# Gadersd/stable-diffusion-xl-burn

Hardware: AMD Instinct MI355X
Metric: images/sec SDXL-base 1024x1024 30-step CFG7.5 (whole job); UNet step ms p50 (higher is better)
Workload: dtype f16; 1 GPU; SDXL-base 1024x1024, n_steps=30 (31 CFG UNet step pairs), CFG 7.5, batch 1 prompt/GPU + VAE decode to u8 (BASELINE configs[1]); precision=f16, vae_dtype=f32_split, weights=synthetic seeded (random-init SDXL-base architecture), mix_classes=0, parallelism=replica x1, 1 prompt per GPU, weights broadcast once over RCCL, hipgraph=True, split_cfg=False, fused_xattn=True, pipelined_decode=False, prompts_per_call=1, full=False, library=stable-diffusion-xl-burn_amd/lib/libsdxl_mi355.so, debug_set=

## Files before the change

stable-diffusion-xl-burn_amd/csrc/capi_ops.hip:

```cpp
#include "capi_internal.h"
#include <algorithm>
#include <cmath>

using namespace sdxl;

namespace {
__global__ void transpose_pad_kernel(const float* src, int lds_, int rows, int C, void* dst, int dt, int ldd) {
  const size_t i = (size_t)blockIdx.x * blockDim.x + threadIdx.x;
  if (i >= (size_t)rows * C) return;
  const int r = i / C, c = i - (size_t)r * C;
  const float v = src[(size_t)r * lds_ + c];
  if (dt == DT_F16) reinterpret_cast<_Float16*>(dst)[(size_t)c * ldd + r] = (_Float16)v;
  else reinterpret_cast<float*>(dst)[(size_t)c * ldd + r] = v;
}
__global__ void causal_mask_kernel(float* out, int n) {
  const int i = blockIdx.x * blockDim.x + threadIdx.x;
  if (i >= n * n) return;
  const int r = i / n, c = i - r * n;
  out[i] = c > r ? -INFINITY : 0.f;
}

struct Operand { std::string name; std::vector<int> shape; int kind; const float* data = nullptr; float eps = 0.f; int ld = 0; };
using Operands = std::vector<Operand>;
void add_linear(Operands& o, const std::string& n, int K, int N, const float* w, const float* b, int ld = 0) {
// ... 249 lines not shown
  SDXL_REQUIRE(ctx && x && gamma && beta && out, "null argument");
  SDXL_REQUIRE(n_group > 0 && C % n_group == 0, "The number of channels must be divisible by the number of groups");
  SDXL_REQUIRE(C % 8 == 0 && n_group <= 256, "unsupported GroupNorm shape");
  use(ctx);
  hipStream_t s = pick(ctx, stream);
  int cdt, sdt; no_mix(dtype); dtypes(dtype, cdt, sdt); no_split(cdt, "sdxl_group_norm");
  Tmp tmp;
  void* xi = tmp.get((size_t)B * HW * C * dt_size(sdt));
  void* yo = tmp.get((size_t)B * HW * C * dt_size(cdt));
  float* part = (float*)tmp.get(groupnorm_workspace_floats(B, n_group) * sizeof(float));
  launch_nchw_to_nhwc(x, C * HW, xi, sdt, B, C, HW, C, 1.0f, s);
  GroupNormParams p{};
  p.X = xi; p.x_dt = sdt; p.ldx = C; p.Y = yo; p.y_dt = cdt; p.ldy = C; p.gamma = gamma; p.beta = beta; p.partial = part;
  p.B = B; p.HW = HW; p.C = C; p.G = n_group; p.eps = eps; p.silu = silu;
  launch_groupnorm(p, s);
  launch_nhwc_to_nchw(yo, cdt, C, out, B, C, HW, 1.0f, s);
  SDXL_HIP(hipStreamSynchronize(s));
  API_END
}
int sdxl_layer_norm(sdxl_ctx* ctx, void* stream, const float* x, const float* gamma, const float* beta, int rows, int C,
                    float eps, int dtype, float* out) {
  API_BEGIN
  SDXL_REQUIRE(ctx && x && gamma && beta && out, "null argument");
  SDXL_REQUIRE(C % 8 == 0, "unsupported LayerNorm width");
  use(ctx);
  hipStream_t s = pick(ctx, stream);
  int cdt, sdt; no_mix(dtype); dtypes(dtype, cdt, sdt); no_split(cdt, "sdxl_layer_norm");
  Tmp tmp;
  void* xi = tmp.get((size_t)rows * C * dt_size(sdt));
  void* yo = tmp.get((size_t)rows * C * dt_size(cdt));
  launch_copy_rows(x, DT_F32, C, xi, sdt, C, rows, C, s);
  LayerNormParams p{};
  p.X = xi; p.x_dt = sdt; p.ldx = C; p.Y = yo; p.y_dt = cdt; p.ldy = C; p.gamma = gamma; p.beta = beta; p.rows = rows; p.C = C; p.eps = eps;
  launch_layernorm(p, s);
  launch_copy_rows(yo, cdt, C, out, DT_F32, C, rows, C, s);
  SDXL_HIP(hipStreamSynchronize(s));
  API_END
}
int sdxl_conv2d(sdxl_ctx* ctx, void* stream, const float* x, const float* weight, const float* bias, int B, int Cin, int H,
                int W, int Cout, int ksize, int stride, int pad, int upsample, int dtype, float* out) {
  API_BEGIN
  SDXL_REQUIRE(ctx && x && weight && out, "null argument");
  use(ctx);
  hipStream_t s = pick(ctx, stream);
  int cdt, sdt;
  if (dtype == SDXL_DTYPE_F32_SPLIT) { cdt = DT_HL; sdt = DT_HL; }
  else { no_mix(dtype); dtypes(dtype, cdt, sdt); }
  SDXL_REQUIRE(cdt != DT_HL || Cin % 32 == 0, "SDXL_DTYPE_F32_SPLIT convolutions need Cin % 32 == 0");
  const int Hs = upsample ? 2 * H : H, Ws = upsample ? 2 * W : W;
  const int Ho = (Hs + 2 * pad - ksize) / stride + 1, Wo = (Ws + 2 * pad - ksize) / stride + 1;
  Operands ops;
  add_conv(ops, "conv", Cout, Cin, ksize, weight, bias);
  Packed pk(ops, cdt, s);
  const Lin l = pk.wb.conv("conv");
  Tmp tmp;
  void* xi = tmp.get((size_t)B * H * W * Cin * dt_size(sdt));
  float* yo = (float*)tmp.get((size_t)B * Ho * Wo * Cout * sizeof(float));
  Act xa(xi, Cin, sdt);
  if (cdt == DT_HL) {
    float* x32 = (float*)tmp.get((size_t)B * H * W * Cin * sizeof(float));
    float* sc = (float*)tmp.get(hl_scale_floats(B) * sizeof(float));
    launch_nchw_to_nhwc(x, Cin * H * W, x32, DT_F32, B, Cin, H * W, Cin, 1.0f, s);
    launch_f32_to_hl_scaled(x32, Cin, xi, Cin, (size_t)B * H * W, Cin, sc, s, B);
    xa.a_scale = hl_scale_inv(sc, B); xa.a_scale_n = B;
  } else launch_nchw_to_nhwc(x, Cin * H * W, xi, sdt, B, Cin, H * W, Cin, 1.0f, s);
  Exec ex; ex.s = s; ex.cdt = cdt; ex.sdt = sdt;
  give_splitk_ws(ex, tmp, B, Ho * Wo, Cout, s);
  run_conv(ex, l, xa, Cin, ConvGeom{B, H, W, Ho, Wo, ksize, stride, pad, upsample ? 1 : 0}, Act(yo, Cout, DT_F32));
  launch_nhwc_to_nchw(yo, DT_F32, Cout, out, B, Cout, Ho * Wo, 1.0f, s);
  SDXL_HIP(hipStreamSynchronize(s));
  API_END
}
int sdxl_linear(sdxl_ctx* ctx, void* stream, const float* x, const float* weight, const float* bias, int M, int K, int N,
                int geglu, int dtype, float* out) {
  API_BEGIN
  SDXL_REQUIRE(ctx && x && weight && out, "null argument");
  SDXL_REQUIRE(!geglu || (N % 32 == 0), "GEGLU width must be a multiple of 32");
  use(ctx);
  hipStream_t s = pick(ctx, stream);
  int cdt, sdt;
  if (dtype == SDXL_DTYPE_F32_SPLIT) { cdt = DT_HL; sdt = DT_HL; }
  else { no_mix(dtype); dtypes(dtype, cdt, sdt); }
  SDXL_REQUIRE(cdt != DT_HL || K % 32 == 0, "SDXL_DTYPE_F32_SPLIT linear layers need K % 32 == 0");
  Operands ops;
  add_linear(ops, "lin", K, N, weight, bias);
  Packed pk(ops, cdt, s);
  const Lin l = pk.wb.linear("lin", geglu != 0);
  Tmp tmp;
  void* xi = tmp.get((size_t)M * K * dt_size(sdt));
  Act xa(xi, K, sdt);
  if (cdt == DT_HL) {
    float* sc = (float*)tmp.get(hl_scale_floats(1) * sizeof(float));
    launch_f32_to_hl_scaled(x, K, xi, K, (size_t)M, K, sc, s, 1);
    xa.a_scale = hl_scale_inv(sc, 1);
  } else launch_copy_rows(x, DT_F32, K, xi, sdt, K, M, K, s);
  Exec ex; ex.s = s; ex.cdt = cdt; ex.sdt = sdt;
  give_splitk_ws(ex, tmp, 1, M, N, s);
  Epi e; e.act = geglu ? 1 : 0;
  run_linear(ex, l, xa, M, Act(out, geglu ? N / 2 : N, DT_F32), e);
  SDXL_HIP(hipStreamSynchronize(s));
  API_END
}
int sdxl_layer_norm_linear(sdxl_ctx* ctx, void* stream, const float* x, const float* gamma, const float* beta, float eps,
                           const float* weight, const float* bias, int M, int K, int N, int geglu, int dtype, float* out) {
  API_BEGIN
  SDXL_REQUIRE(ctx && x && gamma && beta && weight && out, "null argument");
  SDXL_REQUIRE(!geglu || (N % 32 == 0), "GEGLU width must be a multiple of 32");
// ... 217 lines not shown
```

stable-diffusion-xl-burn_amd/csrc/elementwise.hip:

```cpp
#include "kernels.h"
#include <algorithm>
#include <stdexcept>

namespace sdxl {

typedef _Float16 half_t;
typedef _Float16 half8 __attribute__((ext_vector_type(8)));
typedef float f32x4 __attribute__((ext_vector_type(4)));

__device__ __forceinline__ float ld_f(const void* p, size_t i, int dt) {
  if (dt == DT_HL) { const half_t* b = reinterpret_cast<const half_t*>(p) + ((i >> 4) << 5) + (i & 15); return (float)b[0] + (float)b[16]; }
  return dt == DT_F16 ? (float)reinterpret_cast<const half_t*>(p)[i] : reinterpret_cast<const float*>(p)[i];
}
__device__ __forceinline__ void st_f(void* p, size_t i, int dt, float v) {
  if (dt == DT_HL) {
    half_t* b = reinterpret_cast<half_t*>(p) + ((i >> 4) << 5) + (i & 15);
    const half_t hi = (half_t)v;
    b[0] = hi; b[16] = (half_t)(v - (float)hi);
  } else if (dt == DT_F16) reinterpret_cast<half_t*>(p)[i] = (half_t)v; else reinterpret_cast<float*>(p)[i] = v;
}
__device__ __forceinline__ float silu_f(float x) { return x / (1.0f + expf(-x)); }

template <typename WT>
__global__ __launch_bounds__(256) void gemv_kernel(const GemvParams p, int cols) {
// ... 722 lines not shown
    asm("" : "+v"(w));
    const half_t hi = (half_t)w;
    v = !part ? hi : mode == 0 ? (half_t)((w - (float)hi) * lo_scale) : (half_t)((float)hi / lo_scale);
  }
  dst[i + (size_t)n_offset * 2 * K] = v;
}
void launch_pack_linear_hilo(const float* src, void* dst, int K, int N, int Npad, int geglu, float lo_scale, hipStream_t s, int mode, int n_offset) {
  const size_t total = (size_t)Npad * 2 * K;
  hipLaunchKernelGGL(pack_linear_hilo_kernel, dim3((unsigned)((total + 255) / 256)), dim3(256), 0, s, src, reinterpret_cast<half_t*>(dst), K, N, Npad, geglu, lo_scale, mode, n_offset);
}
__global__ void colsum_packed_kernel(const void* wp, int dt, int Kpad, int nrows, float* cs, const float* kscale, int K, int interleave) {
  const int row = blockIdx.x * 4 + (threadIdx.x >> 6), lane = threadIdx.x & 63;
  if (row >= nrows) return;
  float acc = 0.f;
  if (kscale && interleave) {
    for (int k = lane; k < K; k += 64) acc = fmaf(kscale[k], ld_f(wp, (size_t)row * Kpad + 32 * (k >> 4) + (k & 15), dt), acc);
  } else
  if (kscale) { for (int k = lane; k < K; k += 64) acc = fmaf(kscale[k], ld_f(wp, (size_t)row * Kpad + k, dt), acc); }
  else for (int k = lane; k < Kpad; k += 64) acc += ld_f(wp, (size_t)row * Kpad + k, dt);
#pragma unroll
  for (int o = 32; o > 0; o >>= 1) acc += __shfl_xor(acc, o);
  if (lane == 0) cs[row] = acc;
}
void launch_colsum_packed(const void* wp, int dt, int Kpad, int nrows, float* cs, hipStream_t s, const float* kscale, int K, int interleave) {
  hipLaunchKernelGGL(colsum_packed_kernel, dim3((nrows + 3) / 4), dim3(256), 0, s, wp, dt, Kpad, nrows, cs, kscale, K, interleave);
}
__global__ void beta_dot_kernel(const float* w, const float* beta, const float* bias, float* out, int K, int N) {
  const int n = blockIdx.x * blockDim.x + threadIdx.x;
  if (n >= N) return;
  float acc = bias ? bias[n] : 0.f;
  for (int k = 0; k < K; ++k) acc += beta[k] * w[(size_t)k * N + n];
  out[n] = acc;
}
void launch_beta_dot(const float* w, const float* beta, const float* bias, float* out, int K, int N, hipStream_t s) {
  hipLaunchKernelGGL(beta_dot_kernel, dim3((N + 255) / 256), dim3(256), 0, s, w, beta, bias, out, K, N);
}
__global__ void pack_conv_kernel(const float* src, void* dst, int dt, int Cout, int Cin, int ks, int Kpad, int Npad, float wscale) {
  const size_t i = (size_t)blockIdx.x * blockDim.x + threadIdx.x;
  if (i >= (size_t)Npad * Kpad) return;
  const int n = i / Kpad;
  const int k = i - (size_t)n * Kpad;
  float v = 0.f;
  if (n < Cout && k < ks * ks * Cin) {
    const int tap = k / Cin, c = k - tap * Cin;
    const int ky = tap / ks, kx = tap - ky * ks;
    v = src[(((size_t)n * Cin + c) * ks + ky) * ks + kx] * wscale;
  }
  st_f(dst, i, dt, v);
}
void launch_pack_conv(const float* src, void* dst, int dt, int Cout, int Cin, int ks, int Kpad, int Npad, hipStream_t s, float wscale) {
  const size_t total = (size_t)Npad * Kpad;
  hipLaunchKernelGGL(pack_conv_kernel, dim3((total + 255) / 256), dim3(256), 0, s, src, dst, dt, Cout, Cin, ks, Kpad, Npad, wscale);
}
__global__ void pack_bias_kernel(const float* src, float* dst, int N, int Npad, int geglu, int n_offset) {
  const int i = blockIdx.x * blockDim.x + threadIdx.x;
  if (i >= Npad) return;
  float v = 0.f;
  if (i < N && src) v = src[geglu ? geglu_unpermute(i, N) : i];
  dst[n_offset + i] = v;
}
void launch_pack_bias(const float* src, float* dst, int N, int Npad, int geglu, int n_offset, hipStream_t s) {
  hipLaunchKernelGGL(pack_bias_kernel, dim3((Npad + 255) / 256), dim3(256), 0, s, src, dst, N, Npad, geglu, n_offset);
}

}
```

stable-diffusion-xl-burn_amd/csrc/engine.h:

```cpp
#pragma once
#include "kernels.h"

#include <map>
#include <memory>
#include <stdexcept>
#include <string>
#include <utility>
#include <vector>

namespace sdxl {

struct Error : std::runtime_error {
  explicit Error(const std::string& m) : std::runtime_error(m) {}
};
#define SDXL_HIP(x)                                                                                   \
  do {                                                                                                \
    hipError_t e__ = (x);                                                                             \
    if (e__ != hipSuccess) throw ::sdxl::Error(std::string(#x) + " failed: " + hipGetErrorString(e__)); \
  } while (0)
#define SDXL_REQUIRE(cond, msg)                          \
  do {                                                   \
    if (!(cond)) throw ::sdxl::Error(std::string(msg));  \
  } while (0)

// ... 35 lines not shown
uint64_t fnv1a64(const std::string& s);

struct DeviceArena {
  char* base = nullptr;
  size_t cap = 0, off = 0, peak = 0;
  bool dry = false;
  ~DeviceArena();
  void reserve(size_t bytes);
  void* alloc(size_t bytes);
  size_t mark() const { return off; }
  void reset(size_t m) { off = m; }
};

struct WeightSource {
  virtual ~WeightSource() {}
  virtual void fetch(const ParamSpec& s, size_t index, float* dst_dev, hipStream_t st) = 0;
  virtual bool empty() const { return false; }
};
struct NullSource : WeightSource {
  void fetch(const ParamSpec&, size_t, float*, hipStream_t) override {}
  bool empty() const override { return true; }
};
constexpr float kHiLoScale = 256.0f;
constexpr uint64_t kSeedF16Weights = 1ull << 63;
struct SyntheticSource : WeightSource {
  uint64_t seed;
  explicit SyntheticSource(uint64_t s) : seed(s) {}
  void fetch(const ParamSpec& s, size_t index, float* dst_dev, hipStream_t st) override;
};
struct FlatSource : WeightSource {
  const float* base; std::vector<size_t> offsets;
  FlatSource(const float* b, const std::vector<ParamSpec>& specs);
  void fetch(const ParamSpec& s, size_t index, float* dst_dev, hipStream_t st) override;
};

struct FlatSourceF16 : WeightSource {
  const uint16_t* base; std::vector<size_t> offsets;
  void* stage = nullptr; size_t stage_numel = 0;
  FlatSourceF16(const uint16_t* b, const std::vector<ParamSpec>& specs);
  ~FlatSourceF16() override;
  void fetch(const ParamSpec& s, size_t index, float* dst_dev, hipStream_t st) override;
};

struct Lin {
  const void* w = nullptr; const float* b = nullptr;
  const void* wf = nullptr;
  int N = 0, K = 0, Kpad = 0, Npad = 0, ksize = 1, cin = 0;
  const float* cs = nullptr;
  const float* ln_eps = nullptr;
  int ln_k = 0;
  int k_form = 0;
  int dt = -1;
  const float* acc_scale = nullptr;
};
struct NormW { const float* gamma = nullptr; const float* beta = nullptr; const float* eps = nullptr; int C = 0; };

struct WeightBuilder {
  const std::vector<ParamSpec>& specs;
  std::map<std::string, size_t> index;
  WeightSource& src;
  DeviceArena& arena;
  int dt;
  hipStream_t st;
  float* tmp = nullptr; size_t tmp_numel = 0;
  std::string last_fetched;
  WeightBuilder(const std::vector<ParamSpec>& sp, WeightSource& s, DeviceArena& a, int dtype, hipStream_t stream);
  ~WeightBuilder();
  bool wfrag = true;
  static size_t arena_bound(const std::vector<ParamSpec>& specs, int dt, bool wfrag = true);
  const ParamSpec& spec(const std::string& name, size_t* idx = nullptr) const;
  bool has(const std::string& name) const { return index.count(name) != 0; }
  const float* fetch(const std::string& name);
  Lin linear(const std::string& name, bool geglu = false, int dt_override = -1);
  Lin fused_linear(const std::vector<std::string>& names, int dt_override = -1);
  Lin linear_hilo(const std::string& name, bool geglu, bool dup = false, bool hl_interleave = false);
  float hl_scale(Lin& l, const std::vector<std::string>& weight_names);
  Lin linear_ln(const std::string& name, bool geglu, const std::string& norm, bool xattn_query = false);
  Lin fused_linear_ln(const std::vector<std::string>& names, const std::string& norm);
  Lin fold_ln(const std::vector<std::string>& names, const std::string& norm, bool geglu, int dt_override = -1, bool shadow = false, Lin* plain = nullptr, bool hilo_dup = false,
              bool hl_interleave = false);
  bool all_f16_exact(const std::vector<std::string>& names);
  float* tmp2 = nullptr; size_t tmp2_numel = 0;
  Lin conv(const std::string& name);
  void attach_wfrag(Lin& l, bool fill, bool folded = false);
  NormW norm(const std::string& name);
};

struct Act {
  void* p = nullptr; int ld = 0; int dt = DT_F16;
  const float* gn_part = nullptr; int gn_rt = 0;
  const float* a_scale = nullptr;
  int a_scale_n = 1;
  Act() {}
  Act(void* p_, int ld_, int dt_) : p(p_), ld(ld_), dt(dt_) {}
  Act cols(int c0) const { Act a((char*)p + (size_t)c0 * dt_size(dt), ld, dt); a.a_scale = a_scale; a.a_scale_n = a_scale_n; return a; }
};

struct Profiler {
  enum { IGEMM = 0, ATTENTION = 1, GROUPNORM = 2, LAYERNORM = 3, OTHER = 4, NCLS = 5 };
  struct Rec { hipEvent_t a, b; int cls; double flops; int m, n, k, ks, tag; };
  std::vector<Rec> recs;
  void begin(int cls, double flops, hipStream_t s, int m = 0, int n = 0, int k = 0, int ks = 0, int tag = 0);
  void end(hipStream_t s);
  void collect(float ms[NCLS], int launches[NCLS], double flops[NCLS]);
};

struct WarmSeq {
  struct Item { const void* w; unsigned bytes; bool host; unsigned budget; const void* warm[3]; unsigned warm_bytes[3]; };
  std::vector<Item> seq;
  size_t pos = 0;
  bool recording = false, ready = false;
  void finish();
};
struct Exec {
  Profiler* prof = nullptr;
  hipStream_t s = nullptr;
  bool dry = false;
  int cdt = DT_F16;
  int sdt = DT_F16;
  DeviceArena* act = nullptr;
  float* gn_partial = nullptr;
  float* splitk_ws = nullptr; size_t splitk_ws_bytes = 0; unsigned* splitk_cnt = nullptr;
  const float* ebias = nullptr;
  int b0 = 0;
  hipEvent_t fork_ev = nullptr;
  int fork_after = 0, launches = 0;
  WarmSeq* warm = nullptr;
  float* attn_xws = nullptr; unsigned* attn_xcnt = nullptr;
  int demote = 0;
  Act alloc(size_t rows, int C, int dt) {
    return Act(act->alloc(rows * (size_t)C * dt_size(dt)), C, dt);
  }
};

enum MixClass {
  MIX_ATTN_F16 = 1,
// ... 285 lines not shown
```

stable-diffusion-xl-burn_amd/csrc/igemm_common.h:

```cpp
#pragma once
#include "kernels.h"
#include <stdexcept>
#include <type_traits>

namespace sdxl {

typedef _Float16 half_t;
typedef _Float16 half8 __attribute__((ext_vector_type(8)));
typedef _Float16 half4 __attribute__((ext_vector_type(4)));
typedef float f32x4 __attribute__((ext_vector_type(4)));
typedef float f32x16 __attribute__((ext_vector_type(16)));

typedef const __attribute__((address_space(1))) void* gptr_t;
typedef float f32x8 __attribute__((ext_vector_type(8)));
__device__ __forceinline__ f32x8 uniform_load8(const float* ptr) {
  const unsigned long long a = (unsigned long long)(uintptr_t)ptr;
  const unsigned long long u = ((unsigned long long)__builtin_amdgcn_readfirstlane((unsigned)(a >> 32)) << 32) | (unsigned)__builtin_amdgcn_readfirstlane((unsigned)a);
  return *(const __attribute__((address_space(4))) f32x8*)(uintptr_t)u;
}
__device__ __forceinline__ f32x4 col_vec4(const float* arr, bool present, int nbu, int fh, const void* zeros) {
  const f32x8 c = uniform_load8(present ? arr + nbu : reinterpret_cast<const float*>(zeros));
  return fh ? f32x4{c[4], c[5], c[6], c[7]} : f32x4{c[0], c[1], c[2], c[3]};
}
typedef __attribute__((address_space(3))) void* lptr_t;
// ... 67 lines not shown
  static constexpr int TPR = NT / BM;
  static constexpr bool OK = NT % BM == 0 && (TPR == 2 || TPR == 4);
  static constexpr int NC = OK ? 4 / TPR : 1, PERC = 6;
  ln_f32x2 v[NC][PERC];
  int row, sub;
  bool live;
  __device__ __forceinline__ void load(const IgemmParams& p, int m0, int tid) {
    row = tid / TPR; sub = tid - row * TPR;
    const int m = m0 + row;
    live = p.ln_stat != nullptr && p.ln_slots <= 24;
    const ln_f32x2* st = reinterpret_cast<const ln_f32x2*>(p.ln_stat) + (m < p.M ? m : 0);
    const size_t M = (size_t)p.M;
#pragma unroll
    for (int c = 0; c < NC; ++c)
#pragma unroll
      for (int q = 0; q < PERC; ++q) {
        const int k = sub + c * TPR + 4 * q;
        v[c][q] = (live && k < p.ln_slots) ? st[(size_t)k * M] : ln_f32x2{0.f, 0.f};
      }
  }
  __device__ __forceinline__ static float combine(const float (&P)[NC]) {
    if constexpr (TPR == 4) { const float t = P[0] + __shfl_xor(P[0], 1); return t + __shfl_xor(t, 2); }
    else { const float u = P[0] + __shfl_xor(P[0], 1), w = P[1] + __shfl_xor(P[1], 1); return u + w; }
  }
  __device__ __forceinline__ void finish(const IgemmParams& p, int m0, float* coef) {
    if (!live) return;
    float P[NC];
#pragma unroll
    for (int c = 0; c < NC; ++c) {
      P[c] = 0.f;
#pragma unroll
      for (int q = 0; q < PERC; ++q) if (sub + c * TPR + 4 * q < p.ln_slots) P[c] += v[c][q][0];
    }
    const float mu = combine(P) / (float)p.ln_slots;
    float Q[NC], D[NC];
#pragma unroll
    for (int c = 0; c < NC; ++c) {
      Q[c] = 0.f; D[c] = 0.f;
#pragma unroll
      for (int q = 0; q < PERC; ++q)
        if (sub + c * TPR + 4 * q < p.ln_slots) { const float d = v[c][q][0] - mu; Q[c] += v[c][q][1]; D[c] = fmaf(d, d, D[c]); }
    }
    const float s2 = combine(Q), sd = combine(D);
    const float var = (s2 + 64.f * sd) * p.ln_invc;
    const float a = 1.0f / sqrtf(var + (p.ln_eps_ptr ? *p.ln_eps_ptr : p.ln_eps));
    if (sub == 0) {
      const bool ok = m0 + row < p.M;
      coef[row * 2] = ok ? a : 1.f;
      coef[row * 2 + 1] = ok ? -a * mu : 0.f;
    }
  }
};

template <int TM, int TN>
__device__ __forceinline__ void igemm_epilogue(const IgemmParams& p, const f32x16 (&acc)[TM][TN], int mw, int nw, int fr, int fh,
                                               const float (&lnA)[TM], const float (&lnC)[TM]) {
  const bool geglu = p.act == 1;
  const int nlim = geglu ? (p.N >> 1) : p.N;
#pragma unroll
  for (int i = 0; i < TM; ++i) {
    const int m = mw + i * 32 + fr;
    if (m >= p.M) continue;
    const int bidx = m / p.rpb;
    const int key = m - bidx * p.rpb;
    const float lna = lnA[i], lnc = lnC[i];
#pragma unroll
    for (int j = 0; j < TN; ++j) {
      const int nt = nw + j * 32;
#pragma unroll
      for (int q = 0; q < 4; ++q) {
        if (geglu && q >= 2) continue;
        const int nb = nt + 8 * q + 4 * fh;
        if (nb >= p.N) continue;
        float v[4];
#pragma unroll
        for (int r = 0; r < 4; ++r) v[r] = acc[i][j][q * 4 + r];
        if (p.ln_stat) {
          const f32x4 cz = *reinterpret_cast<const f32x4*>(p.ln_cs + nb);
#pragma unroll
          for (int r = 0; r < 4; ++r) v[r] = lna * v[r] + lnc * cz[r];
        }
        if (p.bias) {
          const f32x4 bz = *reinterpret_cast<const f32x4*>(p.bias + nb);
#pragma unroll
          for (int r = 0; r < 4; ++r) v[r] += bz[r];
        }
        if (p.ebias) {
          const f32x4 ez = *reinterpret_cast<const f32x4*>(p.ebias + (size_t)bidx * p.ebias_ld + nb);
#pragma unroll
          for (int r = 0; r < 4; ++r) v[r] += ez[r];
        }
        int nout = nb;
        if (geglu) {
          f32x4 gz = {0.f, 0.f, 0.f, 0.f};
          if (p.bias) gz = *reinterpret_cast<const f32x4*>(p.bias + nb + 16);
          f32x4 gc = {0.f, 0.f, 0.f, 0.f};
          if (p.ln_stat) gc = *reinterpret_cast<const f32x4*>(p.ln_cs + nb + 16);
#pragma unroll
          for (int r = 0; r < 4; ++r) v[r] *= gelu_erf2(lna * acc[i][j][(q + 2) * 4 + r] + lnc * gc[r] + gz[r]);
          nout = (nt >> 1) + 8 * q + 4 * fh;
        }
        if (geglu || nb < p.n_split) {
          const bool vec = nout + 3 < nlim && (nout & 3) == 0;
          if (p.R) {
            if (vec && p.r_dt == DT_F16 && (p.ldr & 3) == 0) {
              const half4 rr = *reinterpret_cast<const half4*>(reinterpret_cast<const half_t*>(p.R) + (size_t)m * p.ldr + nout);
// ... 11 lines not shown
                                           : reinterpret_cast<const float*>(p.R)[(size_t)m * p.ldr + nout + r];
            }
          }
          if (vec && p.c_dt == DT_F16 && (p.ldc & 3) == 0) {
            half4 h; h[0] = (half_t)v[0]; h[1] = (half_t)v[1]; h[2] = (half_t)v[2]; h[3] = (half_t)v[3];
            *reinterpret_cast<half4*>(reinterpret_cast<half_t*>(p.C) + (size_t)m * p.ldc + nout) = h;
          } else if (vec && p.c_dt == DT_F32 && (p.ldc & 3) == 0) {
            f32x4 o = {v[0], v[1], v[2], v[3]};
            *reinterpret_cast<f32x4*>(reinterpret_cast<float*>(p.C) + (size_t)m * p.ldc + nout) = o;
          } else {
#pragma unroll
            for (int r = 0; r < 4; ++r)
              if (nout + r < nlim) {
                if (p.c_dt == DT_F16) reinterpret_cast<half_t*>(p.C)[(size_t)m * p.ldc + nout + r] = (half_t)v[r];
                else reinterpret_cast<float*>(p.C)[(size_t)m * p.ldc + nout + r] = v[r];
              }
          }
        } else {
#pragma unroll
          for (int r = 0; r < 4; ++r)
            if (nb + r < p.N) {
              const size_t o = ((size_t)bidx * p.ct_rows + (nb + r - p.n_split)) * p.ct_ld + key;
              if (p.c_dt == DT_F16) reinterpret_cast<half_t*>(p.Ct)[o] = (half_t)v[r];
              else reinterpret_cast<float*>(p.Ct)[o] = v[r];
            }
        }
      }
    }
  }
}

__host__ __device__ constexpr int pipe_lds_total(int ring, int extra) { return ring + extra + 2048 <= 163840 ? ring + extra + 2048 : ring + extra; }

typedef int warm_i32x4 __attribute__((ext_vector_type(4)));
template <int NT>
__device__ __forceinline__ void igemm_warm_body(const void* base, unsigned bytes, int wi, int nw) {
  const char* b = reinterpret_cast<const char*>(base);
  constexpr unsigned span = NT * 16, step = span * 8;
  warm_i32x4 acc = {0, 0, 0, 0};
  for (size_t off = (size_t)wi * step; off < bytes; off += (size_t)nw * step) {
    warm_i32x4 v[8];
#pragma unroll
    for (int u = 0; u < 8; ++u) {
      const size_t o = off + (size_t)u * span + (size_t)threadIdx.x * 16;
      v[u] = o + 16 <= bytes ? *reinterpret_cast<const warm_i32x4*>(b + o) : warm_i32x4{0, 0, 0, 0};
    }
#pragma unroll
    for (int u = 0; u < 8; ++u) acc ^= v[u];
  }
  asm volatile("" ::"v"(acc));
}

struct GnCtx { char* scratch; int wave, wm, wn, m0, n0; };
template <int TM, int TN, bool GEGLU>
__device__ __forceinline__ void igemm_epilogue_staged_impl(const IgemmParams& p, const f32x16 (&acc)[TM][TN], int mw, int nw,
                                                           int lane, char* lds, bool transposed, const float (&lnA)[TM],
                                                           const float (&lnC)[TM], const void* zeros, const GnCtx* gc = nullptr) {
  constexpr int WM = TM * 32, WN = TN * 32;
  constexpr int ROWS = WM;
  constexpr int COLS = GEGLU ? WN / 2 : WN;
  constexpr int SWN = (COLS % 32) == 0 ? 7 : 0;
  constexpr int SWT = (WM % 32) == 0 ? 7 : 0;
  const int fr = lane & 31, fh = lane >> 5;
  const f32x4* zv = reinterpret_cast<const f32x4*>(zeros);
  constexpr int NQ = GEGLU ? 2 : 4;
  if (!transposed) {
    constexpr int RB = COLS * 4;
    int bidx[TM];
#pragma unroll
    for (int i = 0; i < TM; ++i) { const int m = mw + i * 32 + fr; bidx[i] = (p.ebias && m < p.M) ? m / p.rpb : 0; }
#pragma unroll
    for (int j = 0; j < TN; ++j) {
      const int nt = nw + j * 32;
      f32x4 bz[NQ], cz[NQ], gz[NQ], gc[NQ], ez[TM][NQ];
#pragma unroll
      for (int q = 0; q < NQ; ++q) {
        const int nb = nt + 8 * q + 4 * fh;
        const bool ok = nb < p.N;
        bz[q] = *((p.bias && ok) ? reinterpret_cast<const f32x4*>(p.bias + nb) : zv);
        cz[q] = *((p.ln_stat && ok) ? reinterpret_cast<const f32x4*>(p.ln_cs + nb) : zv);
        if constexpr (GEGLU) {
          gz[q] = *((p.bias && ok) ? reinterpret_cast<const f32x4*>(p.bias + nb + 16) : zv);
          gc[q] = *((p.ln_stat && ok) ? reinterpret_cast<const f32x4*>(p.ln_cs + nb + 16) : zv);
        }
#pragma unroll
        for (int i = 0; i < TM; ++i)
          ez[i][q] = *((p.ebias && ok) ? reinterpret_cast<const f32x4*>(p.ebias + (size_t)bidx[i] * p.ebias_ld + nb) : zv);
      }
#pragma unroll
      for (int i = 0; i < TM; ++i) {
        const int row = i * 32 + fr;
        const float lna = lnA[i], lnc = lnC[i];
#pragma unroll
        for (int q = 0; q < NQ; ++q) {
          f32x4 v;
#pragma unroll
          for (int r = 0; r < 4; ++r) v[r] = acc[i][j][q * 4 + r];
          v = lna * v + lnc * cz[q] + bz[q] + ez[i][q];
          int col = j * 32 + 8 * q + 4 * fh;
          if constexpr (GEGLU) {
#pragma unroll
            for (int r = 0; r < 4; ++r) v[r] *= gelu_erf2(lna * acc[i][j][(q + 2) * 4 + r] + lnc * gc[q][r] + gz[q][r]);
            col = j * 16 + 8 * q + 4 * fh;
          }
          *reinterpret_cast<f32x4*>(lds + row * RB + ((((col >> 2) ^ (row & SWN))) << 4)) = v;
        }
      }
    }
  } else {
    constexpr int RB = WM * 4;
// ... 65 lines not shown
    for (int it = 0; it < NIT; ++it) {
      const int idx = it * 64 + lane;
      const int row = idx / LPR, piece = idx - row * LPR;
      const int n0 = nwo + piece * 8;
      const int m = mw + row;
      const half_t* rp = reinterpret_cast<const half_t*>(p.R) + (size_t)m * p.ldr + n0;
      rfast[it] = p.R && p.r_dt == DT_F16 && idx < ITEMS && m < p.M && n0 + 8 <= nlim && (reinterpret_cast<uintptr_t>(rp) & 15) == 0;
      rpre[it] = *(rfast[it] ? reinterpret_cast<const half8*>(rp) : reinterpret_cast<const half8*>(zeros));
    }
#pragma unroll
    for (int it = 0; it < NIT; ++it) {
      const int idx = it * 64 + lane;
      const int row = idx / LPR, piece = idx - row * LPR;
      if (ITEMS % 64 != 0 && idx >= ITEMS) continue;
      const int n0 = nwo + piece * 8;
      const int m = mw + row;
      const f32x4 a = *reinterpret_cast<const f32x4*>(lds + row * RB + (((2 * piece) ^ (row & SWN)) << 4));
      const f32x4 b = *reinterpret_cast<const f32x4*>(lds + row * RB + (((2 * piece + 1) ^ (row & SWN)) << 4));
      const bool valid = m < p.M && n0 < nlim;
      float rr[8] = {0.f, 0.f, 0.f, 0.f, 0.f, 0.f, 0.f, 0.f};
      if (valid) {
      float v[8] = {a[0], a[1], a[2], a[3], b[0], b[1], b[2], b[3]};
      const bool full = n0 + 8 <= nlim;
      if (rfast[it]) {
#pragma unroll
        for (int e = 0; e < 8; ++e) v[e] += (float)rpre[it][e];
      } else if (p.R) {
        if (p.r_dt == DT_F16) {
          const half_t* rp = reinterpret_cast<const half_t*>(p.R) + (size_t)m * p.ldr + n0;
          if (full && (reinterpret_cast<uintptr_t>(rp) & 15) == 0) {
            const half8 rr = *reinterpret_cast<const half8*>(rp);
#pragma unroll
            for (int e = 0; e < 8; ++e) v[e] += (float)rr[e];
          } else {
#pragma unroll
            for (int e = 0; e < 8; ++e) if (n0 + e < nlim) v[e] += (float)rp[e];
          }
        } else {
          const float* rp = reinterpret_cast<const float*>(p.R) + (size_t)m * p.ldr + n0;
          if (full && (reinterpret_cast<uintptr_t>(rp) & 15) == 0) {
            const f32x4 r0 = *reinterpret_cast<const f32x4*>(rp), r1 = *reinterpret_cast<const f32x4*>(rp + 4);
#pragma unroll
            for (int e = 0; e < 4; ++e) { v[e] += r0[e]; v[4 + e] += r1[e]; }
          } else {
#pragma unroll
            for (int e = 0; e < 8; ++e) if (n0 + e < nlim) v[e] += rp[e];
          }
        }
      }
      if (p.stat_out || gnp) {
#pragma unroll
        for (int e = 0; e < 8; ++e) rr[e] = p.c_dt == DT_F16 ? (float)(half_t)v[e] : v[e];
      }
      if (p.c_dt == DT_F16) {
        half_t* cp = reinterpret_cast<half_t*>(p.C) + (size_t)m * p.ldc + n0;
        if (full && (reinterpret_cast<uintptr_t>(cp) & 15) == 0) {
          half8 h;
#pragma unroll
          for (int e = 0; e < 8; ++e) h[e] = (half_t)v[e];
          *reinterpret_cast<half8*>(cp) = h;
        } else {
#pragma unroll
          for (int e = 0; e < 8; ++e) if (n0 + e < nlim) cp[e] = (half_t)v[e];
        }
      } else if (p.c_dt == DT_HL) {
        if (full) store_hl8(reinterpret_cast<float*>(p.C) + (size_t)m * p.ldc, n0, v);
      } else {
        float* cp = reinterpret_cast<float*>(p.C) + (size_t)m * p.ldc + n0;
        if (full && (reinterpret_cast<uintptr_t>(cp) & 15) == 0) {
          *reinterpret_cast<f32x4*>(cp) = f32x4{v[0], v[1], v[2], v[3]};
          *reinterpret_cast<f32x4*>(cp + 4) = f32x4{v[4], v[5], v[6], v[7]};
        } else {
#pragma unroll
          for (int e = 0; e < 8; ++e) if (n0 + e < nlim) cp[e] = v[e];
        }
      }
      }
      if constexpr (GNP) {
        if (gnp) {
          if (it == 0) {
#pragma unroll
            for (int e = 0; e < 8; ++e) gpiv[e] = __shfl(rr[e], lane & 7);
          }
#pragma unroll
          for (int e = 0; e < 8; ++e) { const float d = rr[e] - gpiv[e]; gs1[e] += d; gs2[e] = fmaf(d, d, gs2[e]); }
        }
      }
      if constexpr (COLS % 64 == 0) {
        if (p.stat_out) {
          const float piv = __shfl(rr[0], lane & ~7);
          float s1 = 0.f, s2 = 0.f;
#pragma unroll
          for (int e = 0; e < 8; ++e) { const float d = rr[e] - piv; s1 += d; s2 = fmaf(d, d, s2); }
          st_piv[it] = piv; st_s1[it] = s1; st_s2[it] = s2;
          st_ok[it] = (piece & 7) == 0 && valid;
          st_off[it] = ((size_t)(n0 >> 6) * p.M + m) * 2;
        }
      }
    }
    if constexpr (COLS % 64 == 0) {
      if (p.stat_out) {
#pragma unroll
        for (int o = 1; o < 8; o <<= 1) {
#pragma unroll
          for (int it = 0; it < NIT; ++it) { st_s1[it] += __shfl_xor(st_s1[it], o); st_s2[it] += __shfl_xor(st_s2[it], o); }
        }
#pragma unroll
        for (int it = 0; it < NIT; ++it)
          if (st_ok[it]) {
            float* dst = p.stat_out + st_off[it];
            dst[0] = st_piv[it] + st_s1[it] * (1.0f / 64.0f);
            dst[1] = fmaxf(st_s2[it] - st_s1[it] * st_s1[it] * (1.0f / 64.0f), 0.f);
          }
      }
    }
    if constexpr (GNP) {
      if (gnp) {
#pragma unroll
        for (int e = 0; e < 8; ++e) {
#pragma unroll
          for (int o = 8; o < 64; o <<= 1) { gs1[e] += __shfl_xor(gs1[e], o); gs2[e] += __shfl_xor(gs2[e], o); }
// ... 225 lines not shown
          dst[1] = fmaxf(s2 - s1 * s1 * (1.0f / 64.0f), 0.f);
        }
      }
    }
  }
}

template <int TM, int TN>
__device__ __forceinline__ void igemm_epilogue_swapped(const IgemmParams& p, const f32x16 (&acc)[TM][TN], int mw, int nw, int lane,
                                                       const float* coef, const void* zeros) {
  (void)zeros;
  const int fr = lane & 31, fh = lane >> 5;
  const int b = mw / p.rpb;
  const int key_w = mw - b * p.rpb;
#pragma unroll
  for (int j = 0; j < TN; ++j) {
    const int n = nw + j * 32 + fr;
    const float bias = p.bias ? p.bias[n] : 0.f;
    const float cs = p.ln_stat ? p.ln_cs[n] : 0.f;
    half_t* crow = reinterpret_cast<half_t*>(p.Ct) + ((size_t)b * p.ct_rows + (n - p.n_split)) * p.ct_ld + key_w;
#pragma unroll
    for (int i = 0; i < TM; ++i) {
      f32x4 v[4];
#pragma unroll
      for (int g = 0; g < 4; ++g) {
        f32x4 a4 = {1.f, 1.f, 1.f, 1.f}, c4 = {0.f, 0.f, 0.f, 0.f};
        if (coef && p.ln_stat) {
          const f32x4 c01 = *reinterpret_cast<const f32x4*>(coef + (i * 32 + 8 * g + 4 * fh) * 2);
          const f32x4 c23 = *reinterpret_cast<const f32x4*>(coef + (i * 32 + 8 * g + 4 * fh) * 2 + 4);
          a4 = f32x4{c01[0], c01[2], c23[0], c23[2]};
          c4 = f32x4{c01[1], c01[3], c23[1], c23[3]};
        }
#pragma unroll
        for (int r = 0; r < 4; ++r) v[g][r] = __builtin_fmaf(a4[r], acc[i][j][4 * g + r], __builtin_fmaf(c4[r], cs, bias));
      }
#pragma unroll
      for (int t = 0; t < 2; ++t) {
        float w[8];
#pragma unroll
        for (int r = 0; r < 4; ++r) {
          const auto sw = __builtin_amdgcn_permlane32_swap(__float_as_uint(v[2 * t][r]), __float_as_uint(v[2 * t + 1][r]), false, false);
          w[r] = __uint_as_float(sw[0]);
          w[4 + r] = __uint_as_float(sw[1]);
        }
        half8 h;
#pragma unroll
        for (int e = 0; e < 8; ++e) h[e] = (half_t)w[e];
        if (n < p.N) *reinterpret_cast<half8*>(crow + i * 32 + 16 * t + 8 * fh) = h;
      }
    }
  }
}

template <int TM, int TN>
__device__ __forceinline__ void igemm_epilogue_staged(const IgemmParams& p, const f32x16 (&acc)[TM][TN], int mw, int nw,
                                                      int lane, char* lds, const float (&lnA)[TM], const float (&lnC)[TM],
                                                      const void* zeros, const GnCtx* gc = nullptr) {
  constexpr int WN = TN * 32;
  if (p.act == 1) { igemm_epilogue_staged_impl<TM, TN, true>(p, acc, mw, nw, lane, lds, false, lnA, lnC, zeros); return; }
  const bool all_normal = nw + WN <= p.n_split || p.n_split >= p.N;
  const bool all_transposed = nw >= p.n_split;
  if (all_normal) igemm_epilogue_staged_impl<TM, TN, false>(p, acc, mw, nw, lane, lds, false, lnA, lnC, zeros, gc);
  else if (all_transposed) igemm_epilogue_staged_impl<TM, TN, false>(p, acc, mw, nw, lane, lds, true, lnA, lnC, zeros);
  else igemm_epilogue<TM, TN>(p, acc, mw, nw, lane & 31, lane >> 5, lnA, lnC);
}

template <int N, typename F> __device__ __forceinline__ void static_for(F&& f) {
  if constexpr (N > 0) {
    static_for<N - 1>(f);
    f(std::integral_constant<int, N - 1>{});
  }
}
template <int OFF, typename F = half8> __device__ __forceinline__ F lds_read128(unsigned addr) {
  F v;
  asm volatile("ds_read_b128 %0, %1 offset:%2" : "=v"(v) : "v"(addr), "n"(OFF));
  return v;
}
template <typename T> struct PipeElem;
template <> struct PipeElem<half_t> {
  typedef half8 frag;
  static __device__ __forceinline__ f32x16 mma(const half8& w, const half8& a, const f32x16& c) {
    return __builtin_amdgcn_mfma_f32_32x32x16_f16(w, a, c, 0, 0, 0);
  }
};
template <> struct PipeElem<float> {
  typedef f32x4 frag;
  static __device__ __forceinline__ f32x16 mma(const f32x4& w, const f32x4& a, f32x16 c) {
    c = __builtin_amdgcn_mfma_f32_32x32x2f32(w[0], a[0], c, 0, 0, 0);
    c = __builtin_amdgcn_mfma_f32_32x32x2f32(w[1], a[1], c, 0, 0, 0);
    c = __builtin_amdgcn_mfma_f32_32x32x2f32(w[2], a[2], c, 0, 0, 0);
    c = __builtin_amdgcn_mfma_f32_32x32x2f32(w[3], a[3], c, 0, 0, 0);
    return c;
  }
};
template <> struct PipeElem<hl16_t> { typedef half8 frag; };
template <int N> __device__ __forceinline__ void wait_lgkmcnt() {
  asm volatile("s_waitcnt lgkmcnt(%0)" ::"n"(N) : "memory");
  __builtin_amdgcn_sched_barrier(0);
}

__device__ __forceinline__ void xattn_load_frags(const IgemmParams& p, int mw, int nw, int lane, half8 (&kf)[3][4], half8 (&vf)[2][6]) {
  const int mclamp = mw < p.M ? mw : p.M - 1;
  const int b = __builtin_amdgcn_readfirstlane(mclamp / p.rpb);
  const int head = (nw < p.N ? nw : 0) >> 6;
  const half8* fx = reinterpret_cast<const half8*>(p.xa_k) + ((size_t)b * (p.N >> 6) + head) * (24 * 64) + lane;
#pragma unroll
  for (int t = 0; t < 3; ++t)
#pragma unroll
    for (int s4 = 0; s4 < 4; ++s4) kf[t][s4] = fx[(t * 4 + s4) * 64];
#pragma unroll
  for (int dt = 0; dt < 2; ++dt)
// ... 237 lines not shown
```

stable-diffusion-xl-burn_amd/csrc/igemm_glds.hip:

```cpp
#include "igemm_common.h"
#include <atomic>

namespace sdxl {

template <int BM, int BN, int NS, int MINB = 2>
__global__ __launch_bounds__(256, MINB) void igemm_glds_kernel(const IgemmParams p, const void* zeros) {
  kernarg_prefetch<(int)sizeof(IgemmParams) + 8>();
  constexpr int WM = BM / 2, WN = BN / 2;
  constexpr int TM = WM / 32, TN = WN / 32;
  constexpr int AJ = BM / 32, BJ = BN / 32;
  constexpr int PER = AJ + BJ;
  constexpr int KT = 64;
  constexpr int STAGE = (BM + BN) * 128;
  extern __shared__ __attribute__((aligned(16))) char smem[];

  const int tid = threadIdx.x, lane = tid & 63;
  const int wave = __builtin_amdgcn_readfirstlane(tid >> 6);
  const int wm = wave >> 1, wn = wave & 1;

  const int tilesN = (p.N + BN - 1) / BN;
  const int nwg = gridDim.x;
  int bid = blockIdx.x;
  {
    const int q = nwg >> 3, r = nwg & 7, xcd = bid & 7, idx = bid >> 3;
// ... 67 lines not shown
  f32x16 acc[TM][TN];
#pragma unroll
  for (int i = 0; i < TM; ++i)
#pragma unroll
    for (int j = 0; j < TN; ++j)
#pragma unroll
      for (int r = 0; r < 16; ++r) acc[i][j][r] = 0.f;

  const int nk = p.Kpad / KT;
  const int fr = lane & 31, fh = lane >> 5;
#pragma unroll
  for (int s = 0; s < NS - 1; ++s)
    if (s < nk) stage(s);
  float lnA[TM], lnC[TM];
  ln_prologue<TM>(p, m0 + wm * WM, fr, lnA, lnC);
  int cur = 0;
  int nxt = NS - 1;
  for (int kt = 0; kt < nk; ++kt) {
    if (kt + NS - 2 < nk) wait_vmcnt<PER * (NS - 2)>(); else wait_vmcnt<0>();
    asm volatile("" ::: "memory");
    __builtin_amdgcn_s_barrier();
    asm volatile("" ::: "memory");
    if (kt + NS - 1 < nk) stage(nxt);
    const char* a = smem + cur * STAGE;
    const char* b = a + BM * 128;
#pragma unroll
    for (int kk = 0; kk < 4; ++kk) {
      const int ch = kk * 2 + fh;
      half8 fa[TM], fb[TN];
#pragma unroll
      for (int i = 0; i < TM; ++i) {
        const int row = wm * WM + i * 32 + fr;
        fa[i] = *reinterpret_cast<const half8*>(a + row * 128 + ((ch ^ ((row >> 1) & 7)) << 4));
      }
#pragma unroll
      for (int j = 0; j < TN; ++j) {
        const int row = wn * WN + j * 32 + fr;
        fb[j] = *reinterpret_cast<const half8*>(b + row * 128 + ((ch ^ ((row >> 1) & 7)) << 4));
      }
#pragma unroll
      for (int i = 0; i < TM; ++i)
#pragma unroll
        for (int j = 0; j < TN; ++j)
          acc[i][j] = __builtin_amdgcn_mfma_f32_32x32x16_f16(fb[j], fa[i], acc[i][j], 0, 0, 0);
    }
    nxt = cur;
    cur = cur + 1 == NS ? 0 : cur + 1;
  }

  __syncthreads();
  igemm_epilogue_staged<TM, TN>(p, acc, m0 + wm * WM, n0 + wn * WN, lane, smem + wave * (WM * WN * 4), lnA, lnC, zeros);
}

template <int BM, int BN, int NS, int WGM = 4, int NW = 8, typename T = half_t, bool XA = false, bool S2 = false, bool TSW = false, bool XH = false>
__global__ __launch_bounds__(64 * NW) void igemm_pipe_kernel(const IgemmParams p, const void* zeros) {
  kernarg_prefetch<(int)sizeof(IgemmParams) + 8>();
  typedef typename PipeElem<T>::frag frag_t;
  constexpr int CE = 16 / (int)sizeof(T);
  constexpr int WGN = NW / WGM;
  constexpr int WM = BM / WGM, WN = BN / WGN;
  constexpr int TM = WM / 32, TN = WN / 32;
  constexpr int NF = TM + TN;
  constexpr int BPC = BN / 8;
  constexpr int AJ = BM / (8 * NW), BJ = (BPC + NW - 1) / NW;
  constexpr int REM = BPC % NW;
  constexpr int PER = AJ + BJ;
  static_assert(BM % (8 * NW) == 0 && WM % 32 == 0 && WN % 32 == 0 && BN % 8 == 0, "bad tile");
  constexpr int KT = 8 * CE;
  constexpr int STAGE = (BM + BN) * 128;
  constexpr bool LIN = XA;
  static_assert(NS >= 3, "counted-wait pipeline needs a ring of at least 3 slots");
  static_assert(BM * 128 + (TN - 1) * 4096 < 65536, "fragment offsets must fit the ds_read immediate");
  extern __shared__ __attribute__((aligned(16))) char smem[];
  const unsigned lds0 = (unsigned)(uintptr_t)(lptr_t)smem;

  const int tid = threadIdx.x, lane = tid & 63;
  const int wave = __builtin_amdgcn_readfirstlane(tid >> 6);
  const int wm = wave / WGN, wn = wave % WGN;
  const bool lastb = REM == 0 || wave < REM;

  const int tilesN = (p.N + BN - 1) / BN;
  const int tilesM = (p.M + BM - 1) / BM;
  const int nwg = gridDim.x;
  int bid = blockIdx.x;
  {
    const int q = nwg >> 3, r = nwg & 7, xcd = bid & 7, idx = bid >> 3;
    bid = (xcd < r ? xcd * (q + 1) : r * (q + 1) + (xcd - r) * q) + idx;
  }
  const int SK = p.splitk > 1 ? p.splitk : 1;
  const int slice = SK > 1 ? bid % SK : 0;
  if (SK > 1) bid /= SK;
  const int tile_id = bid;
  int tm, tn;
  if ((size_t)p.N * p.K > (size_t)p.M * p.Cin) { tn = bid / tilesM; tm = bid - tn * tilesM; }
  else { tm = bid / tilesN; tn = bid - tm * tilesN; }
  const int m0 = tm * BM, n0 = tn * BN;
  bool tsw_swapped = false;
  if constexpr (TSW) {
    const int ok = n0 >= p.n_split && n0 + BN <= p.N && p.c_dt == DT_F16 && p.act == 0 && !p.epi_staged && (p.rpb % BM) == 0 && m0 + BM <= p.M &&
                   (p.ct_ld & 7) == 0 && (reinterpret_cast<uintptr_t>(p.Ct) & 15) == 0 && (!p.ln_stat || p.ln_slots <= 24);
    tsw_swapped = __builtin_amdgcn_readfirstlane(ok) != 0;
  }
  auto wait_tiles = [&](auto KK) {
    constexpr int k = decltype(KK)::value;
    if constexpr (REM == 0) wait_vmcnt<PER * k>();
    else { if (lastb) wait_vmcnt<PER * k>(); else wait_vmcnt<(PER - 1) * k>(); }
  };

  const int lrow = lane >> 3, slot = lane & 7;
  const T* wptr[BJ];
#pragma unroll
  for (int j = 0; j < BJ; ++j) {
    const int row = (j * NW + wave) * 8 + lrow;
    wptr[j] = reinterpret_cast<const T*>(p.W) + (size_t)(n0 + row) * p.Kpad + (slot ^ ((row >> 1) & 7)) * CE;
  }
  const int nk_all = p.Kpad / KT;
  const int kbeg = SK > 1 ? (int)((long)slice * nk_all / SK) : 0;
  const int nk = SK > 1 ? (int)((long)(slice + 1) * nk_all / SK) - kbeg : nk_all;
  if (kbeg > 0) {
#pragma unroll
    for (int j = 0; j < BJ; ++j) wptr[j] += kbeg * KT;
  }
  constexpr bool B0_EARLY = !LIN;
  if constexpr (B0_EARLY) {
    if (nk > 0) {
      char* lb0 = smem + BM * 128 + wave * 1024;
      static_for<BJ>([&](auto J) {
        constexpr int j = decltype(J)::value;
        if (j < BJ - 1 || lastb) {
          __builtin_amdgcn_global_load_lds((gptr_t)wptr[j], (lptr_t)(lb0 + j * (NW * 1024)), 16, 0, 0);
          wptr[j] += KT;
        }
      });
      __builtin_amdgcn_sched_barrier(0);
    }
  }
  const int HWo = p.Hout * p.Wout;
  const int Hup = p.Hin << p.up, Wup = p.Win << p.up;
  const bool lin_rows = p.ksize == 1 && p.stride == 1 && p.up == 0 && p.pad == 0;
  const bool pow2 = (HWo & (HWo - 1)) == 0 && (p.Wout & (p.Wout - 1)) == 0;
  const int sh_hw = __builtin_ctz((unsigned)HWo | 0x40000000u), sh_w = __builtin_ctz((unsigned)p.Wout | 0x40000000u);
  int rb[AJ], ry[AJ], rx[AJ], rsw[AJ];
#pragma unroll
  for (int j = 0; j < AJ; ++j) {
    const int row = (j * NW + wave) * 8 + lrow;
    const int m = m0 + row;
    rsw[j] = (slot ^ ((row >> 1) & 7)) * CE;
    rb[j] = m < p.M ? m : -1; ry[j] = 0; rx[j] = 0;
    if (!lin_rows) {
      if (m < p.M) {
        int b, rem, oy;
        if (pow2) { b = m >> sh_hw; rem = m & (HWo - 1); oy = rem >> sh_w; }
        else { b = m / HWo; rem = m - b * HWo; oy = rem / p.Wout; }
        rb[j] = b; ry[j] = oy * p.stride - p.pad; rx[j] = (rem - oy * p.Wout) * p.stride - p.pad;
      } else { rb[j] = -1; ry[j] = -(1 << 28); rx[j] = 0; }
    }
  }
  const T* Ag = reinterpret_cast<const T*>(p.A);
  const T* aptr[AJ];
  int aadv[AJ];
  int s_c0 = 0, s_dy = 0, s_dx = 0;
  if (kbeg > 0) {
    const int e0 = kbeg * KT, tap = e0 / p.Cin;
    s_c0 = e0 - tap * p.Cin; s_dy = tap / p.ksize; s_dx = tap - s_dy * p.ksize;
  }
  auto retap = [&]() {
    if (lin_rows) {
#pragma unroll
      for (int j = 0; j < AJ; ++j) {
        const bool ok = rb[j] >= 0 && s_dy == 0;
        aptr[j] = ok ? Ag + (size_t)rb[j] * p.lda + rsw[j] + s_c0 : reinterpret_cast<const T*>(zeros);
        aadv[j] = ok ? KT : 0;
      }
      return;
    }
#pragma unroll
    for (int j = 0; j < AJ; ++j) {
      const int iy = ry[j] + s_dy, ix = rx[j] + s_dx;
      const bool ok = (unsigned)iy < (unsigned)Hup && (unsigned)ix < (unsigned)Wup;
      const size_t off = (((size_t)(rb[j] < 0 ? 0 : rb[j]) * p.Hin + ((ok ? iy : 0) >> p.up)) * p.Win + ((ok ? ix : 0) >> p.up)) * p.lda + rsw[j] + s_c0;
      aptr[j] = ok ? Ag + off : reinterpret_cast<const T*>(zeros);
      aadv[j] = ok ? KT : 0;
    }
  };
  retap();
  unsigned long long abase = 0, wbase = 0;
  unsigned aoff[AJ], woff[BJ];
  if constexpr (LIN) {
    abase = (unsigned long long)(uintptr_t)(Ag + (size_t)m0 * p.lda + (size_t)kbeg * KT);
    wbase = (unsigned long long)(uintptr_t)(reinterpret_cast<const T*>(p.W) + (size_t)n0 * p.Kpad + (size_t)kbeg * KT);
    abase = ((unsigned long long)__builtin_amdgcn_readfirstlane((unsigned)(abase >> 32)) << 32) | (unsigned)__builtin_amdgcn_readfirstlane((unsigned)abase);
    wbase = ((unsigned long long)__builtin_amdgcn_readfirstlane((unsigned)(wbase >> 32)) << 32) | (unsigned)__builtin_amdgcn_readfirstlane((unsigned)wbase);
#pragma unroll
    for (int j = 0; j < AJ; ++j) {
      int row = (j * NW + wave) * 8 + lrow;
      const int sw = (slot ^ ((row >> 1) & 7)) * 16;
      if (m0 + row >= p.M) row = p.M - 1 - m0;
      aoff[j] = (unsigned)row * (unsigned)(p.lda * (int)sizeof(T)) + sw;
    }
#pragma unroll
    for (int j = 0; j < BJ; ++j) {
      const int row = (j * NW + wave) * 8 + lrow;
      woff[j] = (unsigned)row * (unsigned)(p.Kpad * (int)sizeof(T)) + (slot ^ ((row >> 1) & 7)) * 16;
    }
  }
  auto issue = [&](int buf, auto PH) {
    constexpr int ph = decltype(PH)::value;
// ... 241 lines not shown
  if constexpr (HL) {
    wait_lgkmcnt<0>();
    if (hl_wexact) kloop(std::true_type{}); else kloop(std::false_type{});
  } else if constexpr (TSW) {
    wait_lgkmcnt<0>();
    if (tsw_swapped) kloop(std::true_type{}); else kloop(std::false_type{});
  } else kloop(std::false_type{});
  __builtin_amdgcn_s_barrier();
  asm volatile("" ::: "memory");
  if constexpr (BN == 128) {
    if (SK > 1) {
      constexpr int NV = TM * TN * 4;
      f32x4* slab = reinterpret_cast<f32x4*>(p.splitk_ws) + ((size_t)tile_id * SK + slice) * (size_t)(NW * NV * 64);
      static_for<TM * TN>([&](auto X) {
        constexpr int x = decltype(X)::value, i = x / TN, j = x % TN;
#pragma unroll
        for (int q = 0; q < 4; ++q) {
          const f32x4 v = f32x4{acc[i][j][4 * q], acc[i][j][4 * q + 1], acc[i][j][4 * q + 2], acc[i][j][4 * q + 3]};
          f32x4* dst = slab + (size_t)((wave * NV + x * 4 + q) * 64 + lane);
          if (p.splitk_wt) asm volatile("global_store_dwordx4 %0, %1, off sc0 sc1\n\ts_nop 1" ::"v"(dst), "v"(v) : "memory");
          else *dst = v;
        }
      });
      asm volatile("s_waitcnt vmcnt(0)" ::: "memory");
      __syncthreads();
      volatile int* flag = reinterpret_cast<volatile int*>(smem + NS * STAGE - 16);
      if (tid == 0) {
        if (!p.splitk_wt) __builtin_amdgcn_fence(__ATOMIC_RELEASE, "agent");
        asm volatile("s_waitcnt vmcnt(0)" ::: "memory");
        const unsigned t = __hip_atomic_fetch_add(p.splitk_cnt + tile_id, 1u, __ATOMIC_RELAXED, __HIP_MEMORY_SCOPE_AGENT);
        const int last = t == (unsigned)(SK - 1);
        if (last) {
          __hip_atomic_store(p.splitk_cnt + tile_id, 0u, __ATOMIC_RELAXED, __HIP_MEMORY_SCOPE_AGENT);
          __builtin_amdgcn_fence(__ATOMIC_ACQUIRE, "agent");
        }
        *flag = last;
      }
      __syncthreads();
      if (!*flag) return;
      const f32x4* s0 = reinterpret_cast<const f32x4*>(p.splitk_ws) + (size_t)tile_id * SK * (size_t)(NW * NV * 64);
      static_for<TM * TN>([&](auto X) {
        constexpr int x = decltype(X)::value, i = x / TN, j = x % TN;
#pragma unroll
        for (int q = 0; q < 4; ++q) {
          f32x4 sum = s0[(size_t)((wave * NV + x * 4 + q) * 64 + lane)];
          for (int sl = 1; sl < SK; ++sl) sum += s0[(size_t)sl * (NW * NV * 64) + (size_t)((wave * NV + x * 4 + q) * 64 + lane)];
#pragma unroll
          for (int r = 0; r < 4; ++r) acc[i][j][4 * q + r] = sum[r];
        }
      });
      __syncthreads();
    }
  }
  if constexpr (XA) {
    static_assert(TN == 2 && sizeof(T) == 2, "fused cross-attention: wave tile = one 64-wide head, f16");
    static_assert(NW * WM * WN * 4 <= NS * STAGE, "staging regions must fit the dead ring");
    if constexpr (XH) {
      static_assert(!XH || (XA && TM == 1), "split-precision fused cross-attention: XA kernels with one-MFMA-row wave tiles");
      xattn_inplace_hl<TM>(p, acc, m0 + wm * WM, n0 + wn * WN, lane, lnA, lnC, zeros);
    } else {
    if constexpr (!XA_EARLY) xattn_load_frags(p, m0 + wm * WM, n0 + wn * WN, lane, xkf, xvf);
    xattn_inplace<TM>(p, acc, m0 + wm * WM, n0 + wn * WN, lane, lnA, lnC, zeros, xkf, xvf);
    }
    IgemmParams pe = p;
    pe.bias = nullptr; pe.ln_stat = nullptr;
    if (!p.epi_staged && igemm_rows_ok<TM, TN, false>(pe, n0 + wn * WN))
      igemm_epilogue_rows<TM, TN, false>(pe, acc, m0 + wm * WM, n0 + wn * WN, lane, lnA, lnC, zeros);
    else
      igemm_epilogue_staged<TM, TN>(pe, acc, m0 + wm * WM, n0 + wn * WN, lane, smem + wave * (WM * WN * 4), lnA, lnC, zeros);
    return;
  }
  if constexpr (TSW) {
    if (tsw_swapped) {
      igemm_epilogue_swapped<TM, TN>(p, acc, m0 + wm * WM, n0 + wn * WN, lane, ln_coop ? ln_coef + (wm * WM) * 2 : nullptr, zeros);
      return;
    }
  }
  if (!p.epi_staged && p.act != 1 && igemm_rows_ok<TM, TN, false>(p, n0 + wn * WN)) {
    igemm_epilogue_rows<TM, TN, false>(p, acc, m0 + wm * WM, n0 + wn * WN, lane, lnA, lnC, zeros);
    return;
  }
  constexpr bool FITS = NW * WM * WN * 4 <= NS * STAGE;
  if (FITS || p.act == 1) {
    const int region = p.act == 1 ? WM * (WN / 2) * 4 : WM * WN * 4;
    if constexpr (BM == 256 && BN == 128 && NW == 8 && WGM == 4 && (sizeof(T) == 2 || HL)) {
      static_assert(NW * WM * WN * 4 + 4096 <= NS * STAGE, "GroupNorm-statistics scratch must fit behind the staging regions");
      const GnCtx gc{smem + NW * WM * WN * 4, wave, wm, wn, m0, n0};
      igemm_epilogue_staged<TM, TN>(p, acc, m0 + wm * WM, n0 + wn * WN, lane, smem + wave * region, lnA, lnC, zeros, &gc);
    } else
    igemm_epilogue_staged<TM, TN>(p, acc, m0 + wm * WM, n0 + wn * WN, lane, smem + wave * region, lnA, lnC, zeros);
  } else {
    igemm_epilogue<TM, TN>(p, acc, m0 + wm * WM, n0 + wn * WN, fr, fh, lnA, lnC);
  }
}

#ifdef SDXL_MEASURE
__device__ unsigned* g_wide_tl = nullptr;
void igemm_set_wide_timeline(void* buf) {
  unsigned* b = reinterpret_cast<unsigned*>(buf);
  if (hipMemcpyToSymbol(HIP_SYMBOL(g_wide_tl), &b, sizeof(b)) != hipSuccess) throw std::runtime_error("igemm: cannot set the wide-kernel timeline buffer");
}
#define WIDE_STAMP(i) do { wtl[i] = (unsigned)__builtin_amdgcn_s_memtime(); } while (0)
#else
#define WIDE_STAMP(i) do { } while (0)
#endif
template <int NS, bool DB = false>
// ... 177 lines not shown
  }
  WIDE_STAMP(3);
  __builtin_amdgcn_s_barrier();
  asm volatile("" ::: "memory");
  WIDE_STAMP(4);
  if (p.act == 1) {
    char* region = smem + wave * (32 * (WN / 2) * 4);
    {
      const float la1[1] = {lnA[0]}, lc1[1] = {lnC[0]};
      igemm_epilogue_staged_impl<1, TN, true>(p, acc0, m0 + wm * WM, n0 + wn * WN, lane, region, false, la1, lc1, zeros);
    }
    WIDE_STAMP(5);
    {
      const float la1[1] = {lnA[1]}, lc1[1] = {lnC[1]};
      igemm_epilogue_staged_impl<1, TN, true>(p, acc1, m0 + wm * WM + 32, n0 + wn * WN, lane, region, false, la1, lc1, zeros);
    }
  }
#ifdef SDXL_MEASURE
  WIDE_STAMP(6);
  asm volatile("s_waitcnt vmcnt(0)" ::: "memory");
  WIDE_STAMP(7);
  wtl[9] = (unsigned)__builtin_amdgcn_s_memrealtime();
  if (g_wide_tl && lane == 0) {
#pragma unroll
    for (int i = 0; i < 10; ++i) g_wide_tl[((size_t)blockIdx.x * 8 + wave) * 16 + i] = wtl[i];
  }
#endif
}

static const void* g_zero_pages[kMaxDevices] = {};
static int current_device() {
  int d = 0;
  if (hipGetDevice(&d) != hipSuccess || d < 0 || d >= kMaxDevices) throw std::runtime_error("igemm: no current HIP device");
  return d;
}
const void* igemm_zero_page() { return g_zero_pages[current_device()]; }
int igemm_current_device() { return current_device(); }
void igemm_glds_init() {
  const int d = current_device();
  if (g_zero_pages[d]) return;
  void* z = nullptr;
  if (hipMalloc(&z, 4096) != hipSuccess || hipMemset(z, 0, 4096) != hipSuccess)
    throw std::runtime_error("igemm: cannot allocate the zero page");
  g_zero_pages[d] = z;
}

template <int BM, int BN, int NS, int MINB = 2>
static void launch_glds(const IgemmParams& p, const IgemmChoice& c, hipStream_t s) {
  const int dev = current_device();
  set_max_dynamic_lds<&igemm_glds_kernel<BM, BN, NS, MINB>>(c.lds, dev);
  hipLaunchKernelGGL((igemm_glds_kernel<BM, BN, NS, MINB>), dim3(c.grid), dim3(c.block), c.lds, s, p, g_zero_pages[dev]);
}

template <int BM, int BN, int NS, int WGM = 4, int NW = 8, typename T = half_t, bool XA = false, bool S2 = false, bool TSW = false, bool XH = false>
static void launch_pipe(const IgemmParams& p, const IgemmChoice& c, hipStream_t s) {
  if (c.lds != pipe_lds_total(NS * (BM + BN) * 128, 0) || c.block != 64 * NW) throw std::logic_error("igemm: choice and kernel disagree on the LDS layout");
  const int dev = current_device();
  set_max_dynamic_lds<&igemm_pipe_kernel<BM, BN, NS, WGM, NW, T, XA, S2, TSW, XH>>(c.lds, dev);
  if (c.splitk > 1 && (size_t)c.grid * BM * BN * 4 > p.splitk_ws_bytes) throw std::runtime_error("igemm: split-K workspace too small");
  hipLaunchKernelGGL((igemm_pipe_kernel<BM, BN, NS, WGM, NW, T, XA, S2, TSW, XH>), dim3(c.grid), dim3(c.block), c.lds, s, p, g_zero_pages[dev]);
}

static void launch_wide(const IgemmParams& p, const IgemmChoice& c, hipStream_t s) {
  const int dev = current_device();
#ifdef SDXL_MEASURE
  if (c.db) {
    set_max_dynamic_lds<&igemm_wide_kernel<3, true>>(c.lds, dev);
    hipLaunchKernelGGL((igemm_wide_kernel<3, true>), dim3(c.grid), dim3(c.block), c.lds, s, p, g_zero_pages[dev]);
    return;
  }
#endif
  set_max_dynamic_lds<&igemm_wide_kernel<3, false>>(c.lds, dev);
  hipLaunchKernelGGL((igemm_wide_kernel<3, false>), dim3(c.grid), dim3(c.block), c.lds, s, p, g_zero_pages[dev]);
}

__global__ void xattn_pack_kernel(const half_t* K, const half_t* Vt, half8* out, int B, int C, int nctx, int vt_ld) {
  const size_t i = (size_t)blockIdx.x * blockDim.x + threadIdx.x;
  const int H = C >> 6;
  if (i >= (size_t)B * H * 24 * 64) return;
  const int lane = (int)(i & 63), f = (int)((i >> 6) % 24);
  const int bh = (int)(i / (24 * 64)), b = bh / H, h = bh - b * H;
  const int fr = lane & 31, fh = lane >> 5;
  half8 v;
#pragma unroll
  for (int e = 0; e < 8; ++e) {
    const int sub = 8 * (e >> 2) + 4 * fh + (e & 3);
    half_t x = (half_t)0.f;
    if (f < 12) {
      const int key = 32 * (f >> 2) + fr, d = 16 * (f & 3) + sub;
      if (key < nctx) x = K[((size_t)b * nctx + key) * C + h * 64 + d];
    } else {
      const int g = f - 12, d = 32 * (g / 6) + fr, key = 16 * (g % 6) + sub;
      if (key < nctx) x = Vt[((size_t)b * C + h * 64 + d) * vt_ld + key];
    }
    v[e] = x;
  }
  out[i] = v;
}
size_t xattn_pack_bytes(int B, int C) { return (size_t)B * (C / 64) * 24 * 64 * 16; }
void launch_xattn_pack(const void* K, const void* Vt, void* out, int B, int C, int nctx, int vt_ld, hipStream_t s) {
  const size_t n = (size_t)B * (C / 64) * 24 * 64;
  hipLaunchKernelGGL(xattn_pack_kernel, dim3((unsigned)((n + 255) / 256)), dim3(256), 0, s, reinterpret_cast<const half_t*>(K),
                     reinterpret_cast<const half_t*>(Vt), reinterpret_cast<half8*>(out), B, C, nctx, vt_ld);
}

void launch_igemm_dma(const IgemmParams& p, const IgemmChoice& c, hipStream_t s) {
#define PIPE(BM, BN, NS, WGM, NW, T, DT, XA, S2, TSW, XH)                                                                                 \
  if (c.family == IG_PIPE && c.bm == BM && c.bn == BN && c.ns == NS && c.wgm == WGM && c.nw == NW && c.elem == DT && c.xa == XA && c.s2 == S2 && c.tsw == TSW && c.xh == XH) \
    return launch_pipe<BM, BN, NS, WGM, NW, T, XA, S2, TSW, XH>(p, c, s)
  PIPE(96, 128, 3, 3, 6, half_t, DT_F16, true, false, false, true);
  PIPE(128, 128, 4, 4, 8, half_t, DT_F16, true, false, false, true);
  PIPE(256, 128, 3, 4, 8, half_t, DT_F16, true, false, false, false);
  PIPE(128, 128, 4, 4, 8, half_t, DT_F16, true, false, false, false);
  PIPE(128, 128, 5, 4, 8, half_t, DT_F16, true, false, false, false);
  PIPE(96, 128, 3, 3, 6, half_t, DT_F16, true, false, false, false);
  PIPE(256, 128, 3, 4, 8, half_t, DT_F16, false, false, false, false);
  if (c.family == IG_GLDS && c.bm == 128 && c.bn == 128 && c.ns == 2) return launch_glds<128, 128, 2>(p, c, s);
  if (c.family == IG_GLDS && c.bm == 64 && c.bn == 128 && c.ns == 2) return launch_glds<64, 128, 2>(p, c, s);
  PIPE(256, 128, 3, 4, 8, half_t, DT_F16, false, false, true, false);
  PIPE(128, 128, 4, 4, 8, half_t, DT_F16, false, false, false, false);
  PIPE(256, 160, 3, 8, 8, half_t, DT_F16, false, false, false, false);
  PIPE(128, 128, 5, 4, 8, half_t, DT_F16, false, false, false, false);
  PIPE(96, 128, 5, 3, 6, half_t, DT_F16, false, false, false, false);
  PIPE(96, 128, 4, 3, 6, half_t, DT_F16, false, false, false, false);
  PIPE(96, 128, 5, 3, 6, half_t, DT_F16, false, true, false, false);
  PIPE(128, 160, 3, 4, 4, half_t, DT_F16, false, false, false, false);
  if (c.family == IG_WIDE && c.bm == 256 && c.bn == 320 && c.ns == 3) return launch_wide(p, c, s);
  PIPE(256, 128, 3, 4, 8, float, DT_F32, false, false, false, false);
  PIPE(128, 128, 4, 4, 8, float, DT_F32, false, false, false, false);
  PIPE(96, 128, 5, 3, 6, hl16_t, DT_HL, false, false, false, false);
  PIPE(256, 128, 3, 4, 8, hl16_t, DT_HL, false, false, false, false);
  PIPE(128, 160, 3, 4, 4, hl16_t, DT_HL, false, false, false, false);
  PIPE(128, 128, 4, 4, 8, hl16_t, DT_HL, false, false, false, false);
#undef PIPE
  throw std::logic_error("igemm: the selection chose a direct-to-LDS kernel that is not instantiated");
}

}
```

stable-diffusion-xl-burn_amd/csrc/kernels.h:

```cpp
#pragma once
#include <hip/hip_runtime.h>
#include <stdint.h>
#include <stdexcept>

namespace sdxl {

enum DType : int { DT_F32 = 0, DT_F16 = 1, DT_HL = 2 };

static inline size_t dt_size(int dt) { return dt == DT_F16 ? 2 : 4; }

struct IgemmParams {
  const void* A;
  const void* W;
  const void* Wf;
  int a_dt;
  int B, Hin, Win, Cin, lda;
  int Hout, Wout;
  int ksize, stride, pad, up;
  int M, N, K, Kpad;
  const float* bias;
  const float* ebias;
  int ebias_ld;
  int rpb;
  int act;
  const void* R; int ldr; int r_dt;
  void* C; int ldc; int c_dt;
  int n_split;
  void* Ct; int ct_rows; int ct_ld;
  const float* ln_stat; int ln_slots; const float* ln_cs; float ln_invc; float ln_eps;
  const float* ln_eps_ptr;
  float* stat_out; int stat_slots;
  float* splitk_ws; size_t splitk_ws_bytes; unsigned* splitk_cnt; int splitk;
  const void* xa_k; int xa_nctx; float xa_scale;
  const void* xa_k_lo;
  float* gn_part;
  const float* acc_scale;
  const float* a_scale;
  int a_scale_rpb;
  int hl_wexact_ok;
  int xa_vec64;
  const void* warm[3]; unsigned warm_bytes[3];
  int splitk_wt;
  int wreg_xcd2d;
  int epi_staged;
  void* shadow; int shadow_ld; const float* shadow_gamma;
  float shadow_lo_scale;
};
struct SelectKnobs {
  int igemm_variant = 0;
  int igemm_wreg = 1;
  int wreg_xattn = 1;
  int hl_tile96 = 29;
  int igemm_tsw = 1;
  int igemm_unrolled = 1;
  int wide_db = 0;
  int attn_variant = 0;
  int attn_xsplit = 1;
  int zero_page = 0;
};
bool select_knob_set(const char* key, int value);
SelectKnobs select_knobs_snapshot();
enum IgemmFamily : int { IG_NONE = 0, IG_GLDS = 1, IG_PIPE = 2, IG_WIDE = 3, IG_WREG = 4, IG_GENERIC = 5, IG_MEASURE = 6 };
struct IgemmChoice {
  int family;
  int bm, bn, ns;
  int wgm, nw;
  int elem, a_elem;
  int xa, xh, tsw, s2;
  int splitk;
  int mode, db, measure;
  int grid, block, lds;
};
IgemmChoice igemm_select(const IgemmParams& p, int compute_dt, const SelectKnobs& k);
bool igemm_gn_part_ok(const IgemmParams& p, const SelectKnobs& k);
bool igemm_wreg_selected(const IgemmParams& p, const SelectKnobs& k);
bool igemm_wreg_xattn_selected(const IgemmParams& p, const SelectKnobs& k);
bool igemm_xattn_ok(int a_dt, int c_dt, int M, int N, int K, int rpb, int n_ctx);
size_t xattn_pack_bytes(int B, int C);
void launch_xattn_pack(const void* K, const void* Vt, void* out, int B, int C, int n_ctx, int vt_ld, hipStream_t s);
int igemm_splitk_slices(const IgemmParams& p);
size_t igemm_splitk_ws_bytes(int batch, int rows_per_entry, int n_max);
constexpr int kSplitkCounters = 4096;
SelectKnobs igemm_launch_knobs();
void launch_igemm(const IgemmParams& p, int compute_dt, const SelectKnobs& knobs, hipStream_t s);
void launch_igemm(const IgemmParams& p, int compute_dt, hipStream_t s);
void launch_repack_wfrag(const void* w, void* wf, int Npad, int Kpad, hipStream_t s);
void igemm_set_warm(int v);
int igemm_warm_enabled();
void igemm_set_splitk_wt(int v);
void igemm_set_wreg_xcd2d(int v);
void igemm_set_hl_weights_exact(int v);
void igemm_set_xa_vec64(int v);
void igemm_set_epilogue_staged(int v);
#ifdef SDXL_MEASURE
void igemm_set_timeline(void* device_buf);
void igemm_set_wreg_timeline(void* device_buf);
void igemm_set_wide_timeline(void* device_buf);
int igemm_timeline_words();
#endif
constexpr int kMaxDevices = 64;
template <auto Kernel> inline void set_max_dynamic_lds(size_t lds, int dev) {
  static bool done[kMaxDevices] = {};
  if (done[dev]) return;
  if (hipFuncSetAttribute(reinterpret_cast<const void*>(Kernel), hipFuncAttributeMaxDynamicSharedMemorySize, (int)lds) != hipSuccess)
    throw std::runtime_error("hipFuncSetAttribute(MaxDynamicSharedMemorySize) failed");
  done[dev] = true;
}
const void* igemm_zero_page();
int igemm_current_device();
void igemm_glds_init();

constexpr int kHlAbsBlocks = 128;
static inline size_t hl_scale_floats(int nb) { return (size_t)nb * (kHlAbsBlocks + 1); }
static inline float* hl_scale_inv(float* scale_io, int nb) { return scale_io + (size_t)nb * kHlAbsBlocks; }

struct GroupNormParams {
  const void* X; int x_dt; int ldx;
  void* Y; int y_dt; int ldy;
  const float* gamma; const float* beta;
  float* partial;
  int B, HW, C, G;
  float eps;
// ... 79 lines not shown
void launch_f16_to_hl(const void* src, int lds, void* dst, int ldd, size_t rows, int C, hipStream_t s);
void launch_f32_to_f16_pair(const float* src, int lds, void* hi, void* lo, int ld16, size_t rows, int C, hipStream_t s);
void launch_hl_zero_lo(void* dst, int ldd, size_t rows, int C, hipStream_t s);
void launch_round_f16(float* p, size_t n, hipStream_t s);
void launch_i32_to_f32(const int* src, float* dst, int n, hipStream_t s);
void launch_embed_tokens(const int* ids, const void* tok, const void* pos, int w_dt, void* x, int x_dt, int ldx, int B, int S,
                         int C, int n_vocab, hipStream_t s);
void launch_argmax_rows(const int* ids, int* out, int B, int S, hipStream_t s);
void launch_gather_rows(const void* x, int x_dt, int ldx, const int* idx, int S, float* out, int B, int C, hipStream_t s);
void launch_causal_mask(float* out, int n, hipStream_t s);
void launch_conditioning_embedding(const float* pooled, int E, const int* vals, int w, int dim, float* out, int n, hipStream_t s);

struct StepCoef {
  float t; float sqrt_a; float sqrt_1ma;
  union { float sqrt_ap; float c_0; };
  union { float sqrt_1map; float c_x; };
  float cfg;
  union { float sigma; float c_z; };
  float c_1;
};
static_assert(sizeof(StepCoef) == 32, "one table entry is eight floats in both layouts");
constexpr int kSolverDdim = 0, kSolverDpmpp2M = 1;
constexpr uint32_t kDrawInitial = 0;
constexpr uint32_t draw_blend(uint32_t i) { return 1u + 2u * i; }
constexpr uint32_t draw_sigma(uint32_t i) { return 2u + 2u * i; }
constexpr int kMaxSeeds = 8;
struct DdimSeeds { uint64_t v[kMaxSeeds]; };
struct DdimParams {
  float* latent;
  const void* eps; int eps_dt; int eps_ld;
  const StepCoef* table; int* step_idx;
  int n, HW; int use_cfg;
  const float* ref; const unsigned char* mask; const float* step_noise; int n_steps_total;
  int seeded; DdimSeeds seeds;
  void* unet_in; int in_dt; int in_ld; int in_rep;
  float* t_out;
  int solver; float* hist;
};
void launch_ddim_step(const DdimParams& p, int do_update, hipStream_t s);
void launch_seeded_noise(float* out, const uint64_t* seeds, uint32_t draw, int n, int HW, hipStream_t s);
void launch_axpby(float* dst, const float* a, float sa, const float* b, float sb, size_t n, hipStream_t s);
void launch_to_u8_image(const void* src, int dt, int lds, unsigned char* dst, size_t pixels, hipStream_t s);
void launch_from_u8_image(const unsigned char* src, void* dst, int dt, int ldd, size_t pixels, hipStream_t s);

void launch_synth_fill(float* dst, size_t numel, uint64_t key, float scale, float mean, hipStream_t s);
void launch_pack_linear(const float* src, void* dst, int dt, int K, int N, int Kpad, int Npad, int geglu,
                        int n_offset, hipStream_t s, const float* kscale = nullptr,
                        float wscale = 1.0f);
void launch_pack_linear_hilo(const float* src, void* dst, int K, int N, int Npad, int geglu, float lo_scale, hipStream_t s, int mode = 0, int n_offset = 0);
void launch_colsum_packed(const void* wp, int dt, int Kpad, int nrows, float* cs, hipStream_t s, const float* kscale = nullptr, int K = 0, int interleave = 0);
void launch_beta_dot(const float* w, const float* beta, const float* bias, float* out, int K, int N, hipStream_t s);
void launch_pack_conv(const float* src, void* dst, int dt, int Cout, int Cin, int ks, int Kpad, int Npad,
                      hipStream_t s, float wscale = 1.0f);
void launch_absmax(const float* src, size_t n, float* out_dev, hipStream_t s, bool accumulate = false);
void launch_pack_bias(const float* src, float* dst, int N, int Npad, int geglu, int n_offset, hipStream_t s);

}
```

stable-diffusion-xl-burn_amd/csrc/select.cpp:

```cpp
#include "kernels.h"
#include <algorithm>
#include <atomic>
#include <cstring>
#include <stdexcept>

namespace sdxl {

namespace {
struct KnobSlot { const char* key; int SelectKnobs::*field; };
constexpr KnobSlot kKnobSlots[] = {
    {"igemm_variant", &SelectKnobs::igemm_variant}, {"igemm_wreg", &SelectKnobs::igemm_wreg}, {"wreg_xattn", &SelectKnobs::wreg_xattn},
    {"hl_tile96", &SelectKnobs::hl_tile96},         {"igemm_tsw", &SelectKnobs::igemm_tsw},   {"wide_db", &SelectKnobs::wide_db},
    {"attn_variant", &SelectKnobs::attn_variant},   {"attn_xsplit", &SelectKnobs::attn_xsplit},
#ifdef SDXL_MEASURE
    {"igemm_unrolled", &SelectKnobs::igemm_unrolled},
#endif
};
constexpr int kNumKnobs = sizeof(kKnobSlots) / sizeof(kKnobSlots[0]);
struct KnobStore {
  std::atomic<int> v[kNumKnobs];
  KnobStore() { const SelectKnobs d; for (int i = 0; i < kNumKnobs; ++i) v[i] = d.*kKnobSlots[i].field; }
};
KnobStore g_knobs;
}
// ... 52 lines not shown
}

int pick_tile(const IgemmParams& p, std::initializer_list<int> among) {
  const int nk = p.Kpad / 64;
  double best = 1e300;
  int number = 35;
  for (int n : among) {
    const Tile& t = tile(n);
    if (!tile_takes(t, p) || (n == 49 && p.act != 0)) continue;
    const double cost = tile_cost(p.M, p.N, nk, t.bm, t.bn, t.w);
    if (cost < best) { best = cost; number = n; }
  }
  if (number == 36 && nk >= 40) number = 44;
  return number;
}

struct Fill { long t96, t128, t256; double eff128, eff256; };
Fill chip_fill(const IgemmParams& p) {
  const long cols = (p.N + 127) / 128;
  const long t96 = (long)((p.M + 95) / 96) * cols, t128 = (long)((p.M + 127) / 128) * cols, t256 = (long)((p.M + 255) / 256) * cols;
  return {t96, t128, t256, (double)t128 / (double)(((t128 + 255) / 256) * 256), (double)t256 / (double)(((t256 + 255) / 256) * 256)};
}
int fill_tile_256_or_128(const IgemmParams& p) {
  const Fill f = chip_fill(p);
  return f.eff256 >= f.eff128 ? 35 : 36;
}

bool wreg_pair_grid_fits(const IgemmParams& p) {
  const long rows = 2L * (p.rpb > 0 ? p.rpb : p.M);
  return ((rows + 95) / 96) * (long)(p.N / 128) <= 512;
}
int wreg_rows(const IgemmParams& p) { return (long)((p.M + 63) / 64) * (p.N / 128) <= 256 ? 64 : 96; }
bool wreg_takes(const IgemmParams& p, const SelectKnobs& k, bool xa) {
  if (!p.Wf || !k.zero_page || (xa ? !p.xa_k || p.xa_k_lo : p.xa_k != nullptr)) return false;
  if (p.a_dt != DT_F16 || (p.c_dt != DT_F16 && (xa || p.c_dt != DT_F32))) return false;
  if (p.ksize != 1 || p.stride != 1 || p.up != 0 || p.pad != 0 || p.Hin != p.Hout || p.Win != p.Wout) return false;
  if (p.N % 128 != 0 || p.Cin != p.K || p.K != p.Kpad || p.Kpad % 64 != 0 || p.Kpad < 128) return false;
  if (p.act != 0 || p.n_split < p.N || p.gn_part || p.acc_scale || p.ebias) return false;
  if ((p.lda & 7) != 0 || misaligned16(p.A) || (p.ldc & 7) != 0 || misaligned16(p.C)) return false;
  if (xa) return !p.stat_out && !p.R && !p.shadow && p.rpb > 0 && p.rpb % 64 == 0 && p.M % p.rpb == 0 && p.xa_nctx >= 1 && p.xa_nctx <= 96;
  if (p.ln_stat || (p.R && ((p.ldr & 7) != 0 || misaligned16(p.R)))) return false;
  if (p.shadow && (p.c_dt != DT_F32 || !p.shadow_gamma || (p.shadow_ld & (p.shadow_lo_scale < 0.f ? 15 : 7)) != 0 || misaligned16(p.shadow))) return false;
  return true;
}
#ifdef SDXL_MEASURE
struct WregForced { int number, bm, depth, mode; };
constexpr WregForced kWregForced[] = {{61, 128, 2, 0}, {63, 96, 2, 1}, {64, 96, 2, 2}, {65, 96, 2, 3}, {66, 96, 2, 4}, {67, 96, 2, 5}, {68, 96, 3, 0},
    {69, 96, 4, 0}, {70, 96, 2, 6}, {71, 96, 2, 7}, {72, 96, 2, 8}, {73, 96, 2, 16 | 32}, {74, 96, 2, 16 | 32 | 4096}, {75, 96, 2, 16 | 32 | 4096 | 128},
    {76, 96, 2, 16 | 4096}, {77, 96, 2, 4096}};
#endif

void set_geometry(IgemmChoice& c, const IgemmParams& p) {
  const int tilesM = (p.M + c.bm - 1) / c.bm, tilesN = (p.N + c.bn - 1) / c.bn;
  c.grid = tilesM * tilesN * (c.splitk > 1 ? c.splitk : 1);
  switch (c.family) {
    case IG_GLDS: c.block = 256; c.lds = c.ns * (c.bm + c.bn) * 128; break;
    case IG_PIPE: {
      const int ring = c.ns * (c.bm + c.bn) * 128;
      c.block = 64 * c.nw; c.lds = ring + 2048 <= 163840 ? ring + 2048 : ring;
    } break;
    case IG_WIDE: c.block = 512; c.lds = c.ns * (c.bm + c.bn) * 64 + 2048; break;
    case IG_WREG: {
      int warm = 0;
      if (p.warm[0] && p.warm_bytes[0] && c.grid <= 512) {
        const int spare = (c.grid <= 256 ? 256 : 512) - c.grid;
        warm = spare < 8 ? 0 : spare > 64 ? 64 : spare;
      }
      c.grid += warm;
      c.block = 512; c.lds = 2 * (c.ns + 1) * c.bm * 128 + (c.xa ? c.bm * 8 : 0);
    } break;
    case IG_GENERIC: c.block = 256; c.lds = 2 * (c.bm + c.bn) * 128; break;
    default: break;
  }
}
IgemmChoice from_tile(int number, int elem, const IgemmParams& p) {
  const Tile& t = tile(number);
  IgemmChoice c{};
  c.family = t.family; c.bm = t.bm; c.bn = t.bn; c.ns = t.ns; c.wgm = t.wgm; c.nw = t.nw; c.s2 = t.s2; c.elem = elem; c.a_elem = elem; c.splitk = 1;
  set_geometry(c, p);
  return c;
}
IgemmChoice wreg_choice(int bm, int depth, int mode, bool xa, const IgemmParams& p) {
  IgemmChoice c{};
  c.family = IG_WREG; c.bm = bm; c.bn = 128; c.ns = depth; c.nw = 8; c.mode = mode; c.xa = xa; c.elem = c.a_elem = DT_F16; c.splitk = 1;
  set_geometry(c, p);
  return c;
}
IgemmChoice wreg_forced_or_auto(int v, bool xa, const IgemmParams& p) {
#ifdef SDXL_MEASURE
  if (!xa) for (const WregForced& f : kWregForced) if (f.number == v) return wreg_choice(f.bm, f.depth, f.mode, false, p);
#endif
  return wreg_choice(v == 60 ? 96 : v == 62 ? 64 : wreg_rows(p), 2, 0, xa, p);
}

bool select_f16(const IgemmParams& p, int v, const SelectKnobs& k, IgemmChoice& c) {
  if (!k.zero_page) return false;
  if (p.act > 1) return false;
  if (p.a_dt != DT_F16 || (p.Cin % 64) != 0 || (p.lda % 8) != 0 || (p.Kpad % 64) != 0) return false;
  if (misaligned16(p.A)) return false;
  if (p.n_split < p.N && (p.n_split & 3) != 0) return false;
  if (p.ebias && (p.ebias_ld & 3) != 0) return false;
  if (p.stat_out && (v == 2 || v == 5 || v == 19 || v == 38)) return false;
  const bool was_auto = v == 0;
  const int nk = p.Kpad / 64;
  if (p.xa_k) {
    if (p.act != 0 || p.n_split < p.N || p.stat_out || p.R || p.ebias ||
        !igemm_xattn_ok(p.a_dt, p.c_dt, p.M, p.N, p.K, p.rpb, p.xa_nctx))
      throw std::runtime_error("igemm: fused cross-attention needs a plain f16 projection (no residual / split outputs)");
    if (!p.xa_k_lo && p.c_dt != DT_F16) throw std::runtime_error("igemm: the f16 fused cross-attention writes f16 rows");
    const bool forced_pipe = v == 35 || v == 36 || v == 44 || v == 45;
    if (p.xa_k_lo) {
      c = from_tile(pick_tile(p, {36, 45}) == 45 ? 45 : 36, DT_F16, p);
      c.xh = 1;
      if (c.bm == 96) c.ns = 3;
    } else if (!forced_pipe && igemm_wreg_xattn_selected(p, k)) {
      c = wreg_forced_or_auto(v, true, p);
      return true;
    } else {
      c = from_tile(forced_pipe ? v : pick_tile(p, {35, 36, 45}), DT_F16, p);
      if (c.bm == 96) c.ns = 3;
    }
    c.xa = 1;
    set_geometry(c, p);
    return true;
  }
  if (p.gn_part) {
    if (!igemm_gn_part_ok(p, k)) throw std::runtime_error("igemm: GroupNorm statistics requested from a shape the 256x128 epilogue does not take");
    v = 0;
  }
  if (p.shadow) {
    if (!igemm_wreg_selected(p, k)) throw std::runtime_error("igemm: an f16 shadow output needs the weights-in-registers kernel");
// ... 9 lines not shown
    return true;
  }
  if (v == 0) v = p.gn_part ? 35 : pick_tile(p, {35, 36, 45, 38, 49, 26});
#ifdef SDXL_MEASURE
  if (was_auto && !k.igemm_unrolled) {
    if (v == 35) v = 11; else if (v == 36) v = 13; else if (v == 38) v = 19;
  }
#else
  (void)was_auto;
#endif
  const Tile* t = find_tile(v);
  if (!t) {
#ifdef SDXL_MEASURE
    c = IgemmChoice{}; c.family = IG_MEASURE; c.measure = v; c.splitk = 1;
    return true;
#else
    return false;
#endif
  }
  if (!tile_takes(*t, p)) return false;
  c = from_tile(v, DT_F16, p);
  if (v == 35 && p.n_split < p.N && k.igemm_tsw && p.c_dt == DT_F16) c.tsw = 1;
#ifdef SDXL_MEASURE
  if (c.family == IG_WIDE) c.db = k.wide_db != 0;
#endif
  return true;
}

bool select_f32(const IgemmParams& p, const SelectKnobs& k, IgemmChoice& c) {
  if (!k.zero_page) return false;
  if (p.act > 1 || p.ln_stat || p.stat_out) return false;
  if (p.a_dt != DT_F32 || (p.Cin % 32) != 0 || (p.lda % 4) != 0 || (p.Kpad % 32) != 0) return false;
  if (misaligned16(p.A)) return false;
  if (p.n_split < p.N && (p.n_split & 3) != 0) return false;
  if (p.ebias && (p.ebias_ld & 3) != 0) return false;
  c = from_tile(fill_tile_256_or_128(p), DT_F32, p);
  return true;
}

bool select_hl(const IgemmParams& p, const SelectKnobs& k, IgemmChoice& c) {
  if (!k.zero_page) return false;
  if (p.act > 1 || p.ln_stat || p.stat_out || p.xa_k) return false;
  if (p.a_dt != DT_HL || (p.Cin % 32) != 0 || (p.lda % 4) != 0 || (p.Kpad % 32) != 0) return false;
  if (p.gn_part && !igemm_gn_part_ok(p, k)) throw std::runtime_error("igemm: GroupNorm statistics requested from a split-operand shape the 256x128 split-K epilogue does not take");
  if (misaligned16(p.A)) return false;
  if (p.n_split < p.N && (p.n_split & 3) != 0) return false;
  if (p.c_dt == DT_HL) {
    if (p.n_split < p.N && p.n_split != 0 && ((p.n_split & 127) != 0 || p.act != 0)) return false;
    const int nout = p.act == 1 ? (p.N >> 1) : p.N;
    if (p.n_split != 0 && ((nout & 7) != 0 || (p.ldc & 15) != 0 || misaligned16(p.C))) return false;
    if (p.n_split < p.N && ((p.ct_ld & 15) != 0 || (p.rpb & 7) != 0 || (p.M % 8) != 0 || misaligned16(p.Ct))) return false;
  }
  if (p.ebias && (p.ebias_ld & 3) != 0) return false;
  const int t96mode = k.hl_tile96;
  const bool splitk = (t96mode & 16) && igemm_splitk_slices(p) > 1;
  const bool plain160 = p.N % 160 == 0 && p.n_split >= p.N && !p.stat_out && p.act == 0;
  const Fill f = chip_fill(p);
  int number;
  if ((t96mode & 1) && (p.ksize == 1 || (t96mode & 2)) && p.n_split >= p.N && f.t128 < 256 && f.t96 <= 256 && f.t96 > f.t128 && f.eff256 < (double)f.t96 / 256.0 && !splitk) {
    number = 45;
  } else if (splitk) {
    number = 35;
  } else if ((t96mode & 4) && plain160 && p.N % 128 != 0) {
    number = 49;
  } else if ((t96mode & 8) && plain160 &&
             tile_cost(p, p.Kpad / 32, 49) < std::min(tile_cost(p, p.Kpad / 32, 35), tile_cost(p, p.Kpad / 32, 36))) {
    number = 49;
  } else {
    number = fill_tile_256_or_128(p);
  }
  c = from_tile(number, DT_HL, p);
  if (splitk) { c.splitk = igemm_splitk_slices(p); set_geometry(c, p); }
  return true;
}

IgemmChoice select_generic(const IgemmParams& p, int compute_dt) {
  struct Cand { int bm, bn; float eff; };
  const Cand cands[4] = {{128, 128, 1.0f}, {128, 64, 0.85f}, {64, 128, 0.85f}, {64, 64, 0.70f}};
  int best = 0; float best_cost = 1e30f;
  for (int i = 0; i < 4; ++i) {
    if (p.act == 1 && cands[i].bn < 64) continue;
    const long tiles = (long)((p.M + cands[i].bm - 1) / cands[i].bm) * ((p.N + cands[i].bn - 1) / cands[i].bn);
    const int slots = 256 * (cands[i].bm * cands[i].bn >= 128 * 128 ? 2 : 4);
    const long waves = (tiles + slots - 1) / slots;
    const float cost = (float)waves * cands[i].bm * cands[i].bn / cands[i].eff;
    if (cost < best_cost) { best_cost = cost; best = i; }
  }
  IgemmChoice c{};
  c.family = IG_GENERIC; c.bm = cands[best].bm; c.bn = cands[best].bn; c.ns = 2; c.wgm = 2; c.nw = 4; c.splitk = 1;
  c.elem = compute_dt == DT_F16 ? DT_F16 : DT_F32;
  c.a_elem = compute_dt == DT_F16 && p.a_dt == DT_F16 ? DT_F16 : DT_F32;
  set_geometry(c, p);
  return c;
}
}

int igemm_splitk_slices(const IgemmParams& p) {
  if (!p.splitk_ws || !p.splitk_cnt) return 1;
  if (p.act != 0 || p.n_split < p.N || p.ln_stat) return 1;
  const int nk = p.Kpad / 64;
  if (p.rpb <= 0 || p.rpb > 1024 || p.N > 1536 || nk < 160) return 1;
  return p.rpb <= 256 ? 8 : 3;
}
size_t igemm_splitk_ws_bytes(int batch, int rows_per_entry, int n_max) {
  if (n_max > 1536) n_max = 1536;
  const long rows3 = (long)batch * (rows_per_entry < 1024 ? rows_per_entry : 1024), rows8 = (long)batch * (rows_per_entry < 256 ? rows_per_entry : 256);
  const size_t slabs3 = (size_t)((rows3 + 255) / 256) * 3, slabs8 = (size_t)((rows8 + 255) / 256) * 8;
  return (slabs3 > slabs8 ? slabs3 : slabs8) * (size_t)((n_max + 127) / 128) * 256 * 128 * 4;
}

bool igemm_gn_part_ok(const IgemmParams& p, const SelectKnobs& k) {
  const bool hl = p.a_dt == DT_HL;
  const int kt = hl ? 32 : 64;
  if (hl ? p.c_dt != DT_F32 : (p.a_dt != DT_F16 || p.c_dt != DT_F16)) return false;
  if ((p.Cin % kt) != 0 || (p.lda % (kt / 8)) != 0 || (p.Kpad % kt) != 0) return false;
  if (p.act != 0 || p.n_split < p.N || p.stat_out || p.ln_stat || p.xa_k) return false;
  if (p.M % 256 != 0 || p.rpb <= 0 || p.rpb % 256 != 0 || p.N % 64 != 0) return false;
  if (p.ebias && (p.ebias_ld & 3) != 0) return false;
  if (hl) return (p.ldc & 3) == 0 && !misaligned16(p.C) && (k.hl_tile96 & 16) && igemm_splitk_slices(p) > 1;
  if (igemm_splitk_slices(p) > 1) return true;
  IgemmParams q = p;
  q.M = 2 * p.rpb;
  if (pick_tile(q, {35, 36, 45, 38, 26}) != 35) return false;
  const int nk = p.Kpad / 64;
  return p.N % 160 != 0 || tile_cost(q, nk, 35) - tile_cost(q, nk, 49) < 6000.0;
}

bool igemm_xattn_ok(int a_dt, int c_dt, int M, int N, int K, int rpb, int n_ctx) {
  return a_dt == DT_F16 && (c_dt == DT_F16 || c_dt == DT_HL) && M > 0 && N % 64 == 0 && K % 64 == 0 && rpb > 0 && rpb % 64 == 0 && M % rpb == 0 &&
         n_ctx >= 1 && n_ctx <= 96;
}
bool igemm_wreg_selected(const IgemmParams& p, const SelectKnobs& k) { return wreg_takes(p, k, false) && k.igemm_wreg && wreg_pair_grid_fits(p); }
bool igemm_wreg_xattn_selected(const IgemmParams& p, const SelectKnobs& k) {
  return wreg_takes(p, k, true) && k.igemm_wreg && k.wreg_xattn && wreg_pair_grid_fits(p);
}

IgemmChoice igemm_select(const IgemmParams& p, int compute_dt, const SelectKnobs& k) {
  IgemmChoice c{};
  if (p.M <= 0 || p.N <= 0) return c;
  const int v = k.igemm_variant;
  if (compute_dt == DT_F16 && v >= 0 && select_f16(p, v, k, c)) return c;
  if (compute_dt == DT_F16 && v > 0 && select_f16(p, 0, k, c)) return c;
  if (p.shadow && compute_dt != DT_F16) throw std::runtime_error("an f16 shadow output needs an f16 GEMM (weights-in-registers kernel)");
  if (compute_dt == DT_F32 && v >= 0 && select_f32(p, k, c)) return c;
  if (compute_dt == DT_HL) {
    if (select_hl(p, k, c)) return c;
    throw std::runtime_error("split-operand (DT_HL) GEMM: shape / alignment outside the direct-to-LDS pipeline");
  }
  if (p.xa_k) throw std::runtime_error("fused cross-attention needs the f16 direct-to-LDS kernels");
  if (p.shadow) throw std::runtime_error("an f16 shadow output needs the f16 weights-in-registers kernel");
  if (p.gn_part) throw std::runtime_error("GroupNorm statistics from the epilogue (gn_part) need the f16 direct-to-LDS 256x128 kernel");
  if (p.ln_stat || p.stat_out)
    throw std::runtime_error("LayerNorm-folded GEMM (ln_stat / stat_out) needs the f16 direct-to-LDS kernels");
  return select_generic(p, compute_dt);
}

int attention_xsplit_heads(int H) { return H - std::max(1, H * 4 / 5); }
size_t attention_xsplit_counters(int B, int H, int Nq) { return (size_t)B * attention_xsplit_heads(H) * ((Nq + 63) / 64) * 2; }
size_t attention_xsplit_ws_bytes(int B, int H, int Nq) { return attention_xsplit_counters(B, H, Nq) * 2 * (9 * 64 * 4 * sizeof(float)); }

#ifdef SDXL_MEASURE
struct AttnKnockout { int number, ko; };
constexpr AttnKnockout kAttnKnockouts[] = {{11, 1}, {12, 2}, {13, 4}, {14, 8}, {15, 16}, {16, 1 | 4}, {17, 2 | 8}};
#endif

AttnChoice attn_select(const AttnParams& p, const SelectKnobs& k) {
  const int v = k.attn_variant;
  AttnChoice c{};
  c.mix = -1; c.block = 256; c.grid_y = 1;
  const int qb128 = (p.Nq + 127) / 128, qb64 = (p.Nq + 63) / 64;
  const bool aligned = ((p.ldq | p.ldk | p.vt_ld | p.ldo) & 7) == 0 &&
                       ((reinterpret_cast<uintptr_t>(p.Q) | reinterpret_cast<uintptr_t>(p.K) |
                         reinterpret_cast<uintptr_t>(p.Vt) | reinterpret_cast<uintptr_t>(p.O)) & 15) == 0;
  if (p.dt == DT_F16 && (v == 0 || (v >= 2 && v <= 17)) && k.zero_page && aligned && !p.mask) {
    c.lds = 3 * 2 * 64 * 128;
    const bool ks_ok = (p.Nk % 64) == 0 && p.Nk >= 128;
    const bool ks_pick = ks_ok && (v == 6 || ((v == 0 || v == 9) && qb128 * p.H < 256));
    if (ks_ok && v == 7) c.mix = 0;
    else if (ks_ok && v == 8) c.mix = 1;
    else if (ks_ok && v == 0 && !ks_pick && p.H % 5 == 0) c.mix = 0;
    else if (ks_pick && v == 0 && p.xws && p.xcnt && k.attn_xsplit && p.H % 5 == 0 && p.H >= 5 && (p.Nk % 128) == 0 && (p.Nq % 64) == 0) c.mix = 2;
    if (c.mix >= 0) {
      c.kernel = AT_MIX;
      c.big_heads = p.H >= 2 ? std::max(1, p.H * 4 / 5) : 0;
      const int ql = c.mix == 0 ? 128 : 64;
      const int nl = p.B * c.big_heads * ((p.Nq + ql - 1) / ql);
      const int nsm = c.mix == 2 ? p.B * (p.H - c.big_heads) * 2 * ((p.Nq + ql - 1) / ql) : p.B * (p.H - c.big_heads) * ((p.Nq + ql / 2 - 1) / (ql / 2));
      c.grid_x = nl + nsm;
      return c;
    }
    if (ks_pick) {
      c.kernel = AT_KS; c.grid_x = qb64 * p.B * p.H;
      return c;
// ... 19 lines not shown
```

stable-diffusion-xl-burn_amd/csrc/unet.cpp:

```cpp
#include "engine.h"

#include <atomic>
#include <cmath>
#include <cstring>

namespace sdxl {

namespace {
ResBlockW load_res(WeightBuilder& wb, const std::string& p, int cin, int cout, std::vector<std::string>& emb_names,
                   int& emb_off) {
  ResBlockW r;
  r.cin = cin; r.cout = cout;
  r.norm_in = wb.norm(p + ".norm_in");
  r.conv_in = wb.conv(p + ".conv_in");
  r.norm_out = wb.norm(p + ".norm_out");
  r.conv_out = wb.conv(p + ".conv_out");
  r.has_skip = wb.has(p + ".skip_connection.weight");
  if (r.has_skip) r.skip = wb.conv(p + ".skip_connection");
  r.emb_off = emb_off;
  emb_names.push_back(p + ".lin_embed");
  emb_off += cout;
  return r;
}
const std::vector<std::string> kQkv = {".attn1.query", ".attn1.key", ".attn1.value"};
// ... 219 lines not shown
}

void UNet::build_weights(WeightSource& src, hipStream_t st) {
  const std::vector<ParamSpec> specs = unet_param_specs(cfg_);
  std::vector<BlockDesc> inp, out; BlockDesc mid;
  unet_block_plan(cfg_, inp, mid, out);
  std::vector<std::pair<std::string, int>> sts;
  auto has_st = [](const BlockDesc& d) { return d.kind == BK_REST || d.kind == BK_RESTU; };
  for (size_t i = 0; i < inp.size(); ++i) if (has_st(inp[i])) sts.push_back({"input_blocks." + std::to_string(i) + ".transformer", inp[i].depth});
  sts.push_back({"middle_block.transformer", mid.depth});
  for (size_t i = 0; i < out.size(); ++i) if (has_st(out[i])) sts.push_back({"output_blocks." + std::to_string(i) + ".transformer", out[i].depth});
  std::vector<StPlan> plans;
  std::vector<std::string> f16_names;
  auto plan_all = [&]() {
    plans.clear(); f16_names.clear();
    for (const auto& t : sts) {
      plans.push_back(plan_transformer(mix_, cdt_, specs, t.first));
      for (int j = 0; j < t.second; ++j) f16_valued_weights(plans.back(), t.first + ".blocks." + std::to_string(j), f16_names);
    }
  };
  plan_all();
  WeightBuilder wb(specs, src, warena_, cdt_, st);
  if (!mix_knob_ && !wb.all_f16_exact(f16_names)) {
    mix_ = (mix_ & (MIX_ATTN_F16 | MIX_GEGLU_F16)) ? (MIX_ATTN_F16 | MIX_GEGLU_F16 | MIX_GEGLU_HILO) : 0;
    plan_all();
    SDXL_REQUIRE(f16_names.empty(), "the fallback classes pack no parameter as f16 values");
  }
  bool x2 = false;
  attn16_ = cdt_ == DT_F16;
  for (const StPlan& pl : plans) {
    x2 = x2 || pl.qkv == LF_X2 || pl.out1 == LF_X2 || pl.q2 == LF_X2 || pl.out2 == LF_X2 || pl.geglu == LF_X2 || pl.ff == LF_X2;
    attn16_ = attn16_ || pl.attn_f16;
  }
  size_t bound = WeightBuilder::arena_bound(specs, cdt_);
  if (x2)
    for (const ParamSpec& ps : specs) if (ps.kind == PK_LINEAR_W) bound += round_up(ps.shape[1], 128) * round_up((size_t)ps.shape[0], 64) * 4 + 256;
  warena_.reserve(bound);
  const int gv = cdt_ == DT_HL ? DT_F32 : -1;
  lin1_t_ = wb.linear("lin1_time_embed", false, gv);
  lin2_t_ = wb.linear("lin2_time_embed", false, gv);
  lin1_l_ = wb.linear("lin1_label_embed", false, gv);
  lin2_l_ = wb.linear("lin2_label_embed", false, gv);
  std::vector<std::string> emb_names;
  int emb_off = 0;
  size_t sti = 0;
  auto load_block = [&](const std::string& p, const BlockDesc& d) {
    BlockW b; b.d = d;
    switch (d.kind) {
      case BK_CONV: case BK_DOWN: b.conv = wb.conv(p); break;
      case BK_RES: b.res = load_res(wb, p, d.c_in, d.c_out, emb_names, emb_off); break;
      default:
        b.res = load_res(wb, p + ".res", d.c_in, d.c_out, emb_names, emb_off);
        if (d.kind == BK_REST || d.kind == BK_RESTU) b.st = load_st(wb, p + ".transformer", d.c_out, d.n_head, d.depth, fuse_ln_, plans[sti++]);
        if (d.kind == BK_RESTU || d.kind == BK_RESU) b.conv = wb.conv(p + ".upsample.conv");
    }
    return b;
  };
  for (size_t i = 0; i < inp.size(); ++i) inp_.push_back(load_block("input_blocks." + std::to_string(i), inp[i]));
  mid_res1_.d = mid;
  mid_res1_.res = load_res(wb, "middle_block.res1", mid.c_in, mid.c_out, emb_names, emb_off);
  mid_res1_.st = load_st(wb, "middle_block.transformer", mid.c_out, mid.n_head, mid.depth, fuse_ln_, plans[sti++]);
  mid_res2_.d = mid;
  mid_res2_.res = load_res(wb, "middle_block.res2", mid.c_in, mid.c_out, emb_names, emb_off);
  for (size_t i = 0; i < out.size(); ++i) out_.push_back(load_block("output_blocks." + std::to_string(i), out[i]));
  norm_out_ = wb.norm("norm_out");
  conv_out_ = wb.conv("conv_out");
  embcat_ = wb.fused_linear(emb_names, gv);
  emb_total_ = emb_off;
  SDXL_HIP(hipStreamSynchronize(st));
  for (BlockW& b : inp_) if (!b.st.blocks.empty()) st_list_.push_back(&b.st);
  st_list_.push_back(&mid_res1_.st);
  for (BlockW& b : out_) if (!b.st.blocks.empty()) st_list_.push_back(&b.st);
}

void UNet::set_context(const float* context, int n_ctx, const float* label, int B, hipStream_t s) {
  SDXL_REQUIRE(B >= 1 && B <= 8, "batch must be in 1..8");
  const int vt_ld = (int)round_up(n_ctx, 64);
  bool pack_xs = false, pack_xa = false;
  for (const STW* st : st_list_) { pack_xs = pack_xs || st->plan.xattn == XA_SPLIT; pack_xa = pack_xa || st->plan.xattn != XA_LAUNCH; }
  pack_xs = pack_xs && n_ctx <= 96; pack_xa = pack_xa && n_ctx <= 96;
  const int kvdt = attn_dt();
  const int emb = 4 * cfg_.model_channels;
  {
    const int dm = cdt_ == DT_HL ? unet_hl_demote() : 0;
    if (dm != demote_mask_ || (dm && demote_flags_.empty())) { demote_mask_ = dm; apply_demote_weights(s); }
  }
  if (B != ctx_B_ || n_ctx != n_ctx_) {
    if (graph_) { (void)hipGraphExecDestroy(graph_); graph_ = nullptr; plan_runs_ = 0; }
    warm_ = WarmSeq();
    plan_runs_ = 0;
    size_t bytes = 1 << 16;
    for (const STW* st : st_list_)
      bytes += st->blocks.size() * (round_up((size_t)B * n_ctx * st->C * dt_size(kvdt), 256) +
                                    round_up((size_t)B * st->C * vt_ld * dt_size(kvdt), 256) +
                                    (pack_xa ? round_up(xattn_pack_bytes(B, st->C), 256) : 0) + (pack_xs ? round_up(xattn_pack_bytes(B, st->C), 256) : 0) + 768);
    bytes += 3 * round_up((size_t)B * emb * sizeof(float), 256);
    if (cdt_ == DT_HL) bytes += round_up((size_t)B * n_ctx * cfg_.context_dim * 4, 256) + 256;
    if (cdt_ == DT_HL) {
      size_t mx = 0;
      for (const STW* st : st_list_) mx = std::max(mx, round_up((size_t)B * n_ctx * st->C * 4, 256) + round_up((size_t)B * st->C * vt_ld * 4, 256));
      bytes += (pack_xs ? 2 * mx + 1024 : pack_xa ? mx + mx / 2 + 512 : mx) + 512;
    }
    ctx_arena_.reserve(bytes);
    ctx_arena_.off = 0;
    SDXL_HIP(hipMemsetAsync(ctx_arena_.base, 0, bytes, s));
    kv_.clear();
    for (const STW* st : st_list_) {
// ... 539 lines not shown
```

stable-diffusion-xl-burn_amd/csrc/vae.cpp:

```cpp
#include "engine.h"

#include <cmath>

namespace sdxl {

VaeResW Vae::load_res(WeightBuilder& wb, const std::string& p, int cin, int cout) {
  VaeResW r; r.cin = cin; r.cout = cout;
  r.n1 = wb.norm(p + ".norm1"); r.c1 = wb.conv(p + ".conv1");
  r.n2 = wb.norm(p + ".norm2"); r.c2 = wb.conv(p + ".conv2");
  r.has_nin = wb.has(p + ".nin_shortcut.weight");
  if (r.has_nin) r.nin = wb.conv(p + ".nin_shortcut");
  return r;
}
VaeMidW Vae::load_mid(WeightBuilder& wb, const std::string& p, int c) {
  VaeMidW m; m.C = c;
  m.b1 = load_res(wb, p + ".block_1", c, c);
  m.an = wb.norm(p + ".attn.norm");
  m.q = wb.conv(p + ".attn.q"); m.k = wb.conv(p + ".attn.k"); m.v = wb.conv(p + ".attn.v");
  m.proj = wb.conv(p + ".attn.proj_out");
  m.b2 = load_res(wb, p + ".block_2", c, c);
  return m;
}

Vae::Vae(const VaeCfg& cfg, int compute_dt, WeightSource* dec_src, WeightSource* enc_src, hipStream_t st)
    : cfg_(cfg), cdt_(compute_dt) {
  const std::vector<ParamSpec> dspecs = vae_decoder_param_specs(cfg_), especs = vae_encoder_param_specs(cfg_);
  size_t bound = 0;
  if (dec_src) bound += WeightBuilder::arena_bound(dspecs, cdt_, false);
  if (enc_src) bound += WeightBuilder::arena_bound(especs, cdt_, false);
  warena_.reserve(bound + 4096);
  if (dec_src) {
    WeightBuilder wb(dspecs, *dec_src, warena_, cdt_, st);
    wb.wfrag = false;
    post_quant_ = wb.conv("post_quant_conv");
    d_conv_in_ = wb.conv("decoder.conv_in");
    d_mid_ = load_mid(wb, "decoder.mid", cfg_.dec.front().first);
    for (size_t i = 0; i < cfg_.dec.size(); ++i) {
      const std::string p = "decoder.blocks." + std::to_string(i);
      DecBlk b;
      b.r[0] = load_res(wb, p + ".res1", cfg_.dec[i].first, cfg_.dec[i].second);
      b.r[1] = load_res(wb, p + ".res2", cfg_.dec[i].second, cfg_.dec[i].second);
      b.r[2] = load_res(wb, p + ".res3", cfg_.dec[i].second, cfg_.dec[i].second);
      b.has_up = i + 1 != cfg_.dec.size();
      if (b.has_up) b.up = wb.conv(p + ".upsampler");
      d_blocks_.push_back(b);
    }
    d_norm_out_ = wb.norm("decoder.norm_out");
    d_conv_out_ = wb.conv("decoder.conv_out");
    SDXL_HIP(hipStreamSynchronize(st));
    has_dec_ = true;
  }
  if (enc_src) {
    WeightBuilder wb(especs, *enc_src, warena_, cdt_, st);
    wb.wfrag = false;
    e_conv_in_ = wb.conv("encoder.conv_in");
    for (size_t i = 0; i < cfg_.enc.size(); ++i) {
      const std::string p = "encoder.blocks." + std::to_string(i);
      EncBlk b;
      b.r[0] = load_res(wb, p + ".res1", cfg_.enc[i].first, cfg_.enc[i].second);
      b.r[1] = load_res(wb, p + ".res2", cfg_.enc[i].second, cfg_.enc[i].second);
      b.has_down = i + 1 != cfg_.enc.size();
      if (b.has_down) b.down = wb.conv(p + ".downsampler");
      e_blocks_.push_back(b);
    }
    e_mid_ = load_mid(wb, "encoder.mid", cfg_.enc.back().first);
    e_norm_out_ = wb.norm("encoder.norm_out");
    e_conv_out_ = wb.conv("encoder.conv_out");
    quant_ = wb.conv("quant_conv");
    SDXL_HIP(hipStreamSynchronize(st));
    has_enc_ = true;
  }
}
Vae::~Vae() {}

void Vae::res_block(Exec& ex, const VaeResW& w, const Act& x, int B, int H, int W, const Act& out) {
  const size_t mk = ex.act->mark();
  const size_t M = (size_t)B * H * W;
  const ConvGeom g3{B, H, W, H, W, 3, 1, 1, 0}, g1{B, H, W, H, W, 1, 1, 0, 0};
  Act gn1 = ex.alloc(M, w.cin, ex.cdt);
  float* nin_max = nullptr;
  if (w.has_nin && ex.cdt == DT_HL && x.dt == DT_F32 && w.nin.dt != DT_F32 && !x.gn_part && M % (size_t)B == 0)
    nin_max = (float*)ex.act->alloc(hl_scale_floats(B) * sizeof(float));
  run_groupnorm(ex, w.n1, x, B, H * W, gn1, true, cfg_.n_group, nin_max);
  Act h = ex.alloc(M, w.cout, ex.sdt);
  run_conv(ex, w.c1, gn1, w.cin, g3, h);
  Act gn2 = ex.alloc(M, w.cout, ex.cdt);
  run_groupnorm(ex, w.n2, h, B, H * W, gn2, true, cfg_.n_group);
  Epi e;
  if (w.has_nin) { run_conv(ex, w.nin, hl_operand(ex, w.nin, x, M, w.cin, B, nin_max), w.cin, g1, out); e.R = out; }
  else e.R = x;
  run_conv(ex, w.c2, gn2, w.cout, g3, out, e);
  ex.act->reset(mk);
}

void Vae::mid(Exec& ex, const VaeMidW& w, const Act& x, int B, int H, int W) {
  const size_t mk = ex.act->mark();
  const int HW = H * W, C = w.C;
// ... 216 lines not shown
```

stable-diffusion-xl-burn_amd/csrc/weights.cpp:

```cpp
#include "engine.h"

#include <cstdio>
#include <cstdlib>
#include <cstring>
#include <cmath>

namespace sdxl {

DeviceArena::~DeviceArena() { if (base) (void)hipFree(base); }
void DeviceArena::reserve(size_t bytes) {
  if (bytes <= cap && base) return;
  if (base) { SDXL_HIP(hipFree(base)); base = nullptr; }
  SDXL_HIP(hipMalloc((void**)&base, bytes));
  cap = bytes;
}
void* DeviceArena::alloc(size_t bytes) {
  const size_t a = round_up(off, 256);
  off = a + bytes;
  if (off > peak) peak = off;
  if (dry) return (void*)(uintptr_t)(a + 256);
  if (off > cap) throw Error("device arena overflow (" + std::to_string(off) + " > " + std::to_string(cap) + ")");
  return base + a;
}

// ... 27 lines not shown
  if ((seed & kSeedF16Weights) && s.kind != PK_EPS) launch_round_f16(dst, s.numel(), st);
}
FlatSource::FlatSource(const float* b, const std::vector<ParamSpec>& specs) : base(b) {
  size_t o = 0;
  for (const ParamSpec& p : specs) { offsets.push_back(o); o += p.numel(); }
}
void FlatSource::fetch(const ParamSpec& s, size_t index, float* dst, hipStream_t st) {
  SDXL_HIP(hipMemcpyAsync(dst, base + offsets[index], s.numel() * sizeof(float), hipMemcpyDefault, st));
  SDXL_HIP(hipStreamSynchronize(st));
}

FlatSourceF16::FlatSourceF16(const uint16_t* b, const std::vector<ParamSpec>& specs) : base(b) {
  size_t o = 0;
  for (const ParamSpec& p : specs) { offsets.push_back(o); o += p.numel(); if (p.numel() > stage_numel) stage_numel = p.numel(); }
  SDXL_HIP(hipMalloc(&stage, stage_numel * sizeof(uint16_t)));
}
FlatSourceF16::~FlatSourceF16() { if (stage) (void)hipFree(stage); }
static float f16_bits_to_float(uint16_t h) {
  const uint32_t sign = (uint32_t)(h & 0x8000u) << 16, e = (h >> 10) & 31u, m = h & 1023u;
  uint32_t bits;
  if (e == 0) {
    if (m == 0) bits = sign;
    else { int sh = 0; uint32_t mm = m; while (!(mm & 1024u)) { mm <<= 1; ++sh; } bits = sign | ((uint32_t)(113 - sh) << 23) | ((mm & 1023u) << 13); }
  } else if (e == 31) bits = sign | 0x7F800000u | (m << 13);
  else bits = sign | ((e + 112u) << 23) | (m << 13);
  float f; std::memcpy(&f, &bits, 4);
  return f;
}
void FlatSourceF16::fetch(const ParamSpec& s, size_t index, float* dst, hipStream_t st) {
  if (s.kind == PK_EPS) {
    uint16_t h = 0;
    SDXL_HIP(hipMemcpyAsync(&h, base + offsets[index], sizeof(h), hipMemcpyDefault, st));
    SDXL_HIP(hipStreamSynchronize(st));
    const float v = h == 0x00A8u ? 1e-5f : (h == 0x0011u ? 1e-6f : f16_bits_to_float(h));
    SDXL_HIP(hipMemcpyAsync(dst, &v, sizeof(float), hipMemcpyHostToDevice, st));
    SDXL_HIP(hipStreamSynchronize(st));
    return;
  }
  SDXL_HIP(hipMemcpyAsync(stage, base + offsets[index], s.numel() * sizeof(uint16_t), hipMemcpyDefault, st));
  SDXL_HIP(hipStreamSynchronize(st));
  launch_copy_rows(stage, DT_F16, 1, dst, DT_F32, 1, (int)s.numel(), 1, st);
}

WeightBuilder::WeightBuilder(const std::vector<ParamSpec>& sp, WeightSource& s, DeviceArena& a, int dtype, hipStream_t stream)
    : specs(sp), src(s), arena(a), dt(dtype), st(stream) {
  for (size_t i = 0; i < specs.size(); ++i) {
    index[specs[i].name] = i;
    if (specs[i].numel() > tmp_numel) tmp_numel = specs[i].numel();
  }
  SDXL_HIP(hipMalloc((void**)&tmp, tmp_numel * sizeof(float)));
}
WeightBuilder::~WeightBuilder() { if (tmp) (void)hipFree(tmp); if (tmp2) (void)hipFree(tmp2); }

size_t WeightBuilder::arena_bound(const std::vector<ParamSpec>& specs, int dt, bool wfrag) {
  size_t total = 1 << 20;
  for (const ParamSpec& p : specs) {
    if (p.kind == PK_LINEAR_W) total += round_up(p.shape[1], 128) * round_up(p.shape[0], 64) * dt_size(dt) + 768;
    else if (p.kind == PK_CONV_W)
      total += round_up(p.shape[0], 128) * round_up((size_t)p.shape[1] * p.shape[2] * p.shape[3], 64) * dt_size(dt) + 768;
    else total += round_up(p.numel(), 128) * sizeof(float) + 256;
    if (p.kind == PK_LINEAR_W || p.kind == PK_CONV_W) total += round_up(p.kind == PK_LINEAR_W ? p.shape[1] : p.shape[0], 128) * 4 + 256;
    if (p.kind == PK_LINEAR_W) total += round_up(p.shape[1], 128) * 4 + 256;
    if (wfrag && dt == DT_F16 && p.kind == PK_LINEAR_W) total += round_up(p.shape[1], 128) * round_up(p.shape[0], 64) * 2 + 256;
    if (wfrag && dt == DT_F16 && p.kind == PK_CONV_W && p.shape[2] == 1) total += round_up(p.shape[0], 128) * round_up((size_t)p.shape[1], 64) * 2 + 256;
  }
  return total;
}
const ParamSpec& WeightBuilder::spec(const std::string& name, size_t* idx) const {
  auto it = index.find(name);
  if (it == index.end()) throw Error("unknown parameter '" + name + "'");
  if (idx) *idx = it->second;
  return specs[it->second];
}
const float* WeightBuilder::fetch(const std::string& name) {
  if (name == last_fetched) return tmp;
  size_t i; const ParamSpec& s = spec(name, &i);
  src.fetch(s, i, tmp, st);
  last_fetched = name;
  return tmp;
}
float WeightBuilder::hl_scale(Lin& l, const std::vector<std::string>& weight_names) {
  float* sc = (float*)arena.alloc(2 * sizeof(float));
  l.acc_scale = sc;
  if (src.empty()) return 1.f;
  SDXL_HIP(hipMemsetAsync(sc, 0, 2 * sizeof(float), st));
  for (const std::string& n : weight_names) launch_absmax(fetch(n), spec(n).numel(), sc, st, true);
  float h = 0.f;
  SDXL_HIP(hipMemcpyAsync(&h, sc, sizeof(float), hipMemcpyDeviceToHost, st));
  SDXL_HIP(hipStreamSynchronize(st));
  int e = 0;
  if (h > 0.f && std::isfinite(h)) { (void)std::frexp(h, &e); e = 14 - e; }
  e = e > 24 ? 24 : (e < -24 ? -24 : e);
  const float wscale = std::ldexp(1.0f, e), inv = 1.0f / wscale;
  SDXL_HIP(hipMemcpyAsync(sc, &inv, sizeof(float), hipMemcpyHostToDevice, st));
  SDXL_HIP(hipStreamSynchronize(st));
  bool first = true;
  for (const std::string& n : weight_names) { launch_f16_exact(fetch(n), spec(n).numel(), wscale, sc + 1, st, !first); first = false; }
  return wscale;
}

void WeightBuilder::attach_wfrag(Lin& l, bool fill, bool folded) {
  const int wdt = l.dt >= 0 ? l.dt : dt;
  if (!wfrag) return;
  if (wdt != DT_F16 || l.ksize != 1 || l.N % 128 != 0 || l.K != l.Kpad || l.Kpad % 64 != 0 || l.Kpad < 128 || (l.cs && !folded) || l.acc_scale) return;
  void* wf = arena.alloc((size_t)l.Npad * l.Kpad * 2);
  l.wf = wf;
  if (fill) launch_repack_wfrag(l.w, wf, l.Npad, l.Kpad, st);
}
Lin WeightBuilder::linear(const std::string& name, bool geglu, int dt_override) {
  const ParamSpec& s = spec(name + ".weight");
  Lin l; l.K = s.shape[0]; l.N = s.shape[1]; l.ksize = 1; l.cin = l.K;
  const int wdt = dt_override >= 0 ? dt_override : ((dt == DT_HL && l.K % 32 != 0) ? DT_F32 : dt);
  if (wdt != dt) l.dt = wdt;
  const int kt = wdt == DT_F16 ? 64 : 32;
  l.Kpad = (int)round_up(l.K, kt); l.Npad = (int)round_up(l.N, 128);
  void* w = arena.alloc((size_t)l.Npad * l.Kpad * dt_size(wdt));
  float* b = (float*)arena.alloc((size_t)l.Npad * sizeof(float));
  l.w = w; l.b = b;
  const float wscale = wdt == DT_HL ? hl_scale(l, {name + ".weight"}) : 1.f;
  if (src.empty()) { if (!geglu) attach_wfrag(l, false); return l; }
  launch_pack_linear(fetch(name + ".weight"), w, wdt, l.K, l.N, l.Kpad, l.Npad, geglu ? 1 : 0, 0, st, nullptr, wscale);
  const float* bsrc = has(name + ".bias") ? fetch(name + ".bias") : nullptr;
  launch_pack_bias(bsrc, b, l.N, l.Npad, geglu ? 1 : 0, 0, st);
  if (!geglu) attach_wfrag(l, true);
  return l;
}
Lin WeightBuilder::linear_hilo(const std::string& name, bool geglu, bool dup, bool hl_interleave) {
  const ParamSpec& s = spec(name + ".weight");
  const int K0 = s.shape[0];
  SDXL_REQUIRE(K0 % 32 == 0, "linear_hilo: K % 32 == 0");
  Lin l; l.K = 2 * K0; l.N = s.shape[1]; l.ksize = 1; l.cin = l.K; l.dt = DT_F16; l.k_form = hl_interleave ? 2 : 1;
  l.Kpad = l.K; l.Npad = (int)round_up(l.N, 128);
  void* w = arena.alloc((size_t)l.Npad * l.Kpad * 2);
  float* b = (float*)arena.alloc((size_t)l.Npad * sizeof(float));
  l.w = w; l.b = b;
  if (src.empty()) { if (hl_interleave && !geglu) attach_wfrag(l, false); return l; }
  launch_pack_linear_hilo(fetch(name + ".weight"), w, K0, l.N, l.Npad, geglu ? 1 : 0, kHiLoScale, st, hl_interleave ? 2 : dup ? 1 : 0);
  const float* bsrc = has(name + ".bias") ? fetch(name + ".bias") : nullptr;
  launch_pack_bias(bsrc, b, l.N, l.Npad, geglu ? 1 : 0, 0, st);
  if (hl_interleave && !geglu) attach_wfrag(l, true);
  return l;
}
Lin WeightBuilder::fused_linear(const std::vector<std::string>& names, int dt_override) {
  Lin l; l.ksize = 1;
  int ntot = 0;
  for (const std::string& n : names) {
    const ParamSpec& s = spec(n + ".weight");
    if (l.K == 0) l.K = s.shape[0];
// ... 64 lines not shown
  SDXL_REQUIRE(!hilo_dup || (shadow && names.size() == 1 && dt == DT_F16 && l.K % 32 == 0), "fold_ln: the (hi | lo) form is a single f16 shadow-form projection");
  const int K0 = l.K;
  SDXL_REQUIRE(!hl_interleave || (shadow && !hilo_dup && dt == DT_F16 && l.K % 32 == 0), "fold_ln: the HL16-interleaved form is an f16 shadow-form projection");
  if (hilo_dup) { l.ln_k = K0; l.K = 2 * K0; l.k_form = 1; }
  if (hl_interleave) { l.ln_k = K0; l.K = 2 * K0; l.k_form = 2; }
  l.N = ntot; l.cin = l.K;
  const int kt = dt == DT_F16 ? 64 : 32;
  l.Kpad = (int)round_up(l.K, kt); l.Npad = (int)round_up(l.N, 128);
  char* w = (char*)arena.alloc((size_t)l.Npad * l.Kpad * dt_size(dt));
  float* b = (float*)arena.alloc((size_t)l.Npad * sizeof(float));
  float* cs = (float*)arena.alloc((size_t)l.Npad * sizeof(float));
  float* leps = (float*)arena.alloc(sizeof(float));
  l.w = w; l.b = b; l.cs = cs; l.ln_eps = leps;
  float* bplain = plain ? (float*)arena.alloc((size_t)l.Npad * sizeof(float)) : nullptr;
  if (plain) { *plain = l; plain->b = bplain; plain->cs = nullptr; plain->ln_eps = nullptr; }
  if (src.empty()) return l;
  SDXL_HIP(hipMemcpyAsync(leps, fetch(norm + ".eps"), sizeof(float), hipMemcpyDeviceToDevice, st));
  const size_t need = 3 * (size_t)l.Npad + 2 * (size_t)l.K + 64;
  if (need > tmp2_numel) {
    if (tmp2) SDXL_HIP(hipFree(tmp2));
    SDXL_HIP(hipMalloc((void**)&tmp2, need * sizeof(float)));
    tmp2_numel = need;
  }
  float* gamma = tmp2;
  float* beta = tmp2 + l.K;
  float* bsrc = beta + l.K;
  float* bfold = bsrc + l.Npad;
  SDXL_REQUIRE(spec(norm + ".gamma").shape[0] == K0, "fused_linear_ln: norm width mismatch");
  SDXL_HIP(hipMemcpyAsync(gamma, fetch(norm + ".gamma"), K0 * sizeof(float), hipMemcpyDeviceToDevice, st));
  SDXL_HIP(hipMemcpyAsync(beta, fetch(norm + ".beta"), K0 * sizeof(float), hipMemcpyDeviceToDevice, st));
  SDXL_HIP(hipMemsetAsync(w, 0, (size_t)l.Npad * l.Kpad * dt_size(dt), st));
  SDXL_HIP(hipMemsetAsync(b, 0, (size_t)l.Npad * sizeof(float), st));
  if (bplain) SDXL_HIP(hipMemsetAsync(bplain, 0, (size_t)l.Npad * sizeof(float), st));
  int off = 0;
  for (const std::string& n : names) {
    const ParamSpec& s = spec(n + ".weight");
    const int N = s.shape[1];
    const bool hb = has(n + ".bias");
    if (hb) SDXL_HIP(hipMemcpyAsync(bsrc, fetch(n + ".bias"), N * sizeof(float), hipMemcpyDeviceToDevice, st));
    const float* wsrc = fetch(n + ".weight");
    if (hl_interleave) launch_pack_linear_hilo(wsrc, w, K0, N, names.size() == 1 ? l.Npad : N, geglu ? 1 : 0, kHiLoScale, st, 2, off);
    else if (hilo_dup) launch_pack_linear_hilo(wsrc, w, K0, N, l.Npad, geglu ? 1 : 0, kHiLoScale, st, 1);
    else if (names.size() == 1) launch_pack_linear(wsrc, w, dt, l.K, N, l.Kpad, l.Npad, geglu ? 1 : 0, 0, st, shadow ? nullptr : gamma);
    else launch_pack_linear(wsrc, w, dt, l.K, N, l.Kpad, N, 0, off, st, shadow ? nullptr : gamma);
    launch_beta_dot(wsrc, beta, hb ? bsrc : nullptr, bfold, K0, N, st);
    launch_pack_bias(bfold, b, N, names.size() == 1 ? l.Npad : N, geglu ? 1 : 0, off, st);
    if (bplain) launch_pack_bias(hb ? bsrc : nullptr, bplain, N, names.size() == 1 ? l.Npad : N, geglu ? 1 : 0, off, st);
    off += N;
  }
  if (shadow) launch_colsum_packed(w, dt, l.Kpad, l.Npad, cs, st, gamma, K0, hl_interleave ? 1 : 0);
  else launch_colsum_packed(w, dt, l.Kpad, l.Npad, cs, st);
  return l;
}
Lin WeightBuilder::conv(const std::string& name) {
  const ParamSpec& s = spec(name + ".weight");
  Lin l; l.N = s.shape[0]; l.cin = s.shape[1]; l.ksize = s.shape[2];
  l.K = l.cin * l.ksize * l.ksize;
  const int wdt = (dt == DT_HL && l.cin % 32 != 0) ? DT_F32 : dt;
  if (wdt != dt) l.dt = wdt;
  const int kt = wdt == DT_F16 ? 64 : 32;
  l.Kpad = (int)round_up(l.K, kt); l.Npad = (int)round_up(l.N, 128);
  void* w = arena.alloc((size_t)l.Npad * l.Kpad * dt_size(wdt));
  float* b = (float*)arena.alloc((size_t)l.Npad * sizeof(float));
  l.w = w; l.b = b;
  const float wscale = wdt == DT_HL ? hl_scale(l, {name + ".weight"}) : 1.f;
  if (src.empty()) { attach_wfrag(l, false); return l; }
  launch_pack_conv(fetch(name + ".weight"), w, wdt, l.N, l.cin, l.ksize, l.Kpad, l.Npad, st, wscale);
  launch_pack_bias(fetch(name + ".bias"), b, l.N, l.Npad, 0, 0, st);
  attach_wfrag(l, true);
  return l;
}
NormW WeightBuilder::norm(const std::string& name) {
  const ParamSpec& s = spec(name + ".gamma");
  NormW n; n.C = s.shape[0];
  float* g = (float*)arena.alloc((size_t)n.C * sizeof(float));
  float* b = (float*)arena.alloc((size_t)n.C * sizeof(float));
  float* e = (float*)arena.alloc(sizeof(float));
  n.gamma = g; n.beta = b; n.eps = e;
  if (src.empty()) return n;
  SDXL_HIP(hipMemcpyAsync(g, fetch(name + ".gamma"), n.C * sizeof(float), hipMemcpyDeviceToDevice, st));
  SDXL_HIP(hipMemcpyAsync(b, fetch(name + ".beta"), n.C * sizeof(float), hipMemcpyDeviceToDevice, st));
  SDXL_HIP(hipMemcpyAsync(e, fetch(name + ".eps"), sizeof(float), hipMemcpyDeviceToDevice, st));
  return n;
}

void WarmSeq::finish() {
  const size_t n = seq.size();
  for (Item& it : seq) for (int r = 0; r < 3; ++r) { it.warm[r] = nullptr; it.warm_bytes[r] = 0; }
  for (size_t j = 0; j < n && n > 4; ++j) {
    const unsigned bytes = seq[j].bytes;
    if (bytes < (1u << 18) || bytes > (seq[j].host ? 14u << 20 : 8u << 20)) continue;
    for (size_t d = 1; d <= 4; ++d) {
      Item& h = seq[(j + n - d) % n];
      if (!h.host || h.warm[2] || h.w == seq[j].w || h.budget < bytes) continue;
      const int r = !h.warm[0] ? 0 : !h.warm[1] ? 1 : 2;
      h.warm[r] = seq[j].w; h.warm_bytes[r] = bytes;
      h.budget -= bytes;
      break;
    }
  }
  recording = false; ready = true; pos = 0;
  if (std::getenv("SDXL_WARM_DUMP")) {
    std::vector<char> covered(n, 0);
    for (size_t i = 0; i < n; ++i) for (int r = 0; r < 3; ++r) if (seq[i].warm[r]) for (size_t j = 0; j < n; ++j) if (seq[j].w == seq[i].warm[r]) covered[j] = 1;
    size_t tb = 0, cb = 0;
    for (size_t i = 0; i < n; ++i) {
      tb += seq[i].bytes; if (covered[i]) cb += seq[i].bytes;
      std::fprintf(stderr, "[warm] %3zu %9u B %s carries %u + %u + %u B %s\n", i, seq[i].bytes, seq[i].host ? "host" : "    ", seq[i].warm_bytes[0], seq[i].warm_bytes[1],
                   seq[i].warm_bytes[2], covered[i] ? "" : "*");
    }
    std::fprintf(stderr, "[warm] %zu entries, %.1f MB read per forward, %.1f MB of it warmed\n", n, tb / 1048576.0, cb / 1048576.0);
  }
}
bool run_conv(Exec& ex, const Lin& w, const Act& a, int cin, const ConvGeom& g, const Act& out, const Epi& e) {
  if (ex.dry) return false;
  SDXL_REQUIRE(cin == w.cin, "run_conv: channel mismatch");
  IgemmParams p{};
  p.A = a.p; p.W = w.w; p.Wf = w.wf; p.a_dt = a.dt;
  p.B = g.B; p.Hin = g.Hin; p.Win = g.Win; p.Cin = cin; p.lda = a.ld;
  p.Hout = g.Hout; p.Wout = g.Wout;
  p.ksize = g.ksize; p.stride = g.stride; p.pad = g.pad; p.up = g.up;
  p.M = g.B * g.Hout * g.Wout; p.N = w.N; p.K = w.K; p.Kpad = w.Kpad;
  p.bias = w.b; p.ebias = e.ebias; p.ebias_ld = e.ebias_ld;
  p.rpb = e.rpb ? e.rpb : g.Hout * g.Wout;
  p.act = e.act;
  p.R = e.R.p; p.ldr = e.R.ld; p.r_dt = e.R.dt;
  p.C = out.p; p.ldc = out.ld; p.c_dt = out.dt;
  p.n_split = e.n_split >= 0 ? e.n_split : w.N;
  p.Ct = e.Ct; p.ct_rows = e.ct_rows; p.ct_ld = e.ct_ld;
  p.ln_stat = e.ln_stat; p.ln_slots = (w.ln_k ? w.ln_k : w.K) / 64; p.ln_cs = w.cs; p.ln_invc = 1.0f / (float)(w.ln_k ? w.ln_k : w.K); p.ln_eps = 1e-5f; p.ln_eps_ptr = w.ln_eps;
  p.stat_out = e.stat_out; p.stat_slots = w.N / 64;
  p.splitk_ws = ex.splitk_ws; p.splitk_ws_bytes = ex.splitk_ws_bytes; p.splitk_cnt = ex.splitk_cnt; p.splitk = 0;
  p.xa_k = e.xa_k; p.xa_nctx = e.xa_nctx; p.xa_scale = e.xa_scale; p.xa_k_lo = e.xa_k_lo;
  p.acc_scale = w.acc_scale;
  p.a_scale = (w.dt >= 0 ? w.dt : ex.cdt) == DT_HL ? a.a_scale : nullptr;
  p.a_scale_rpb = (p.a_scale && a.a_scale_n > 1) ? p.M / a.a_scale_n : 0;
  const SelectKnobs knobs = igemm_launch_knobs();
  p.gn_part = nullptr;
  {
    const int wdt_ = w.dt >= 0 ? w.dt : ex.cdt;
    if (e.gn_part && (wdt_ == DT_F16 || wdt_ == DT_HL) && wdt_ == ex.cdt) { p.gn_part = e.gn_part; if (!igemm_gn_part_ok(p, knobs)) p.gn_part = nullptr; }
  }
  if (e.shadow_done) *e.shadow_done = false;
  if (e.shadow) {
    p.shadow = e.shadow; p.shadow_ld = e.shadow_ld; p.shadow_gamma = e.shadow_gamma; p.shadow_lo_scale = e.shadow_lo_scale;
    const bool ok = (w.dt >= 0 ? w.dt : ex.cdt) == DT_F16 && igemm_wreg_selected(p, knobs);
    if (!ok) { p.shadow = nullptr; p.shadow_gamma = nullptr; p.stat_out = nullptr; p.shadow_lo_scale = 0.f; }
    if (e.shadow_done) *e.shadow_done = ok;
  }
  SDXL_REQUIRE(!e.xa_k || igemm_xattn_ok(a.dt, out.dt, p.M, p.N, p.K, p.rpb, e.xa_nctx), "fused cross-attention: unsupported shape");
  SDXL_REQUIRE(!e.ln_stat || (w.ln_k ? w.ln_k : w.K) % 64 == 0, "LayerNorm-folded GEMM needs K % 64 == 0");
  SDXL_REQUIRE(!e.stat_out || (w.N % 64 == 0 && (e.n_split < 0 || e.n_split >= w.N) && e.act == 0), "row statistics need a plain N % 64 == 0 output");
  SDXL_REQUIRE(!e.ln_stat || w.cs, "ln_stat given but the weight is not LayerNorm-folded");
  SDXL_REQUIRE(!w.cs || e.ln_stat, "LayerNorm-folded weight used without row statistics");
  SDXL_REQUIRE(!((w.dt >= 0 ? w.dt : ex.cdt) == DT_F32 && a.dt != DT_F32), "f32 compute needs f32 activations");
  if (ex.prof) ex.prof->begin(Profiler::IGEMM, 2.0 * p.M * (double)p.N * p.K, ex.s, p.M, p.N, p.K, p.ksize, e.cls);
  if (ex.warm && (w.dt >= 0 ? w.dt : ex.cdt) == DT_F16) {
    WarmSeq& ws = *ex.warm;
    const bool host = igemm_wreg_selected(p, knobs) || igemm_wreg_xattn_selected(p, knobs);
    const size_t wbytes = (size_t)w.Npad * w.Kpad * 2;
    const char* lo; const char* hi;
    if (host) {
      const char* f = reinterpret_cast<const char*>(p.Wf), *b = reinterpret_cast<const char*>(w.b);
      lo = (b && b < f && f - b <= (64 << 10)) ? b : f;
      hi = f + wbytes;
    } else {
      lo = reinterpret_cast<const char*>(p.W); hi = lo + wbytes;
      auto ext = [&](const void* q, size_t sz) { const char* c = reinterpret_cast<const char*>(q); if (q && c >= hi && c - hi <= (64 << 10)) hi = c + sz; };
      ext(w.b, (size_t)w.Npad * 4); ext(w.cs, (size_t)w.Npad * 4); ext(w.ln_eps, 4);
    }
    if (ws.recording) {
      if (p.xa_k) ws.seq.push_back(WarmSeq::Item{p.xa_k, (unsigned)xattn_pack_bytes(p.M / p.rpb, p.N), false, 0u, {nullptr, nullptr, nullptr}, {0u, 0u, 0u}});
      const unsigned budget = host ? 14u << 20 : 0u;
      ws.seq.push_back(WarmSeq::Item{lo, (unsigned)(hi - lo), host, budget, {nullptr, nullptr, nullptr}, {0u, 0u, 0u}});
    } else if (ws.ready) {
      if (p.xa_k) ++ws.pos;
      if (ws.pos < ws.seq.size()) {
        const WarmSeq::Item& it = ws.seq[ws.pos++];
        if (it.w == lo) for (int r = 0; r < 3; ++r) { p.warm[r] = it.warm[r]; p.warm_bytes[r] = it.warm_bytes[r]; }
      }
    }
  }
  launch_igemm(p, w.dt >= 0 ? w.dt : ex.cdt, knobs, ex.s);
  {
    const hipError_t le = hipGetLastError();
    if (le != hipSuccess)
      throw Error(std::string("implicit-GEMM launch failed (") + hipGetErrorString(le) + "): M=" + std::to_string(p.M) + " N=" + std::to_string(p.N) +
                  " K=" + std::to_string(p.K) + " ksize=" + std::to_string(p.ksize) + " a_dt=" + std::to_string(p.a_dt) + " c_dt=" + std::to_string(p.c_dt) +
                  " compute=" + std::to_string(w.dt >= 0 ? w.dt : ex.cdt) + " act=" + std::to_string(p.act) + " n_split=" + std::to_string(p.n_split));
  }
  if (ex.prof) ex.prof->end(ex.s);
  {
    static const bool nan_check = std::getenv("SDXL_NAN_CHECK") != nullptr;
    hipStreamCaptureStatus cs = hipStreamCaptureStatusNone;
    if (nan_check && hipStreamIsCapturing(ex.s, &cs) == hipSuccess && cs == hipStreamCaptureStatusNone) {
      const int nout = p.act == 1 ? p.N / 2 : (p.n_split < p.N ? p.n_split : p.N);
      const unsigned bo = nout > 0 ? count_nonfinite(out.p, out.dt, out.ld, (size_t)p.M, nout, ex.s) : 0;
      if (bo) {
        const unsigned bi = p.ksize == 1 && p.stride == 1 && !p.up ? count_nonfinite(a.p, a.dt, a.ld, (size_t)p.M, cin, ex.s) : 0;
        std::fprintf(stderr, "[nan] GEMM tag %d M %d N %d K %d ks %d act %d a_dt %d c_dt %d compute %d: %u non-finite outputs, %u non-finite inputs\n", e.cls, p.M, p.N,
                     p.K, p.ksize, p.act, p.a_dt, p.c_dt, w.dt >= 0 ? w.dt : ex.cdt, bo, bi);
      }
    }
  }
  if (ex.fork_ev && ++ex.launches == ex.fork_after) SDXL_HIP(hipEventRecord(ex.fork_ev, ex.s));
  return p.gn_part != nullptr;
}
Act hl_operand(Exec& ex, const Lin& w, const Act& x, size_t rows, int C, int nb, float* have_max) {
  if (ex.cdt != DT_HL || x.dt != DT_F32 || w.dt == DT_F32) return x;
  if (nb < 1 || rows % (size_t)nb != 0) { SDXL_REQUIRE(!have_max, "hl_operand: absmax partials need whole batch entries"); nb = 1; }
  Act o = ex.alloc(rows, C, DT_HL);
  float* sc = have_max ? have_max : (float*)ex.act->alloc(hl_scale_floats(nb) * sizeof(float));
  if (!ex.dry) launch_f32_to_hl_scaled(x.p, x.ld, o.p, o.ld, rows, C, sc, ex.s, nb, have_max != nullptr);
  o.a_scale = hl_scale_inv(sc, nb); o.a_scale_n = nb;
  return o;
}
bool run_linear(Exec& ex, const Lin& w, const Act& a, int M, const Act& out, const Epi& e) {
  ConvGeom g{1, M, 1, M, 1, 1, 1, 0, 0};
  Epi e2 = e;
  if (e2.rpb == 0) e2.rpb = M;
  return run_conv(ex, w, a, w.cin, g, out, e2);
}
void run_groupnorm(Exec& ex, const NormW& n, const Act& x, int B, int HW, const Act& y, bool silu, int groups, float* absmax_out) {
  if (ex.dry) return;
  SDXL_REQUIRE(groups >= 1 && groups <= 256 && n.C % groups == 0, "The number of channels must be divisible by the number of groups");
  GroupNormParams p{};
  p.X = x.p; p.x_dt = x.dt; p.ldx = x.ld;
  p.Y = y.p; p.y_dt = y.dt; p.ldy = y.ld;
  p.gamma = n.gamma; p.beta = n.beta; p.partial = ex.gn_partial;
  p.B = B; p.HW = HW; p.C = n.C; p.G = groups; p.eps = 1e-5f; p.eps_ptr = n.eps; p.silu = silu ? 1 : 0;
  p.chan_part = x.gn_part; p.chan_rt = x.gn_rt; p.chan_rows = 256;
  SDXL_REQUIRE(!absmax_out || (!x.gn_part && x.dt == DT_F32), "GroupNorm absmax side output needs the statistics pass over an fp32 tensor");
  p.absmax_out = absmax_out;
  SDXL_REQUIRE(!x.gn_part || x.gn_rt * 256 == HW, "producer GroupNorm statistics do not cover the tensor");
  {
    static const bool gn_dump = std::getenv("SDXL_GN_DUMP") != nullptr;
    if (gn_dump) std::fprintf(stderr, "[gn] B %d HW %d C %d x_dt %d %s\n", B, HW, n.C, x.dt, x.gn_part ? "producer statistics" : "statistics pass");
  }
  if (ex.prof) ex.prof->begin(Profiler::GROUPNORM, 0.0, ex.s);
  launch_groupnorm(p, ex.s);
  {
    const hipError_t le = hipGetLastError();
    if (le != hipSuccess) throw Error(std::string("GroupNorm launch failed (") + hipGetErrorString(le) + "): C=" + std::to_string(p.C) + " HW=" + std::to_string(p.HW) + " y_dt=" + std::to_string(p.y_dt));
  }
  if (ex.prof) ex.prof->end(ex.s);
}
void run_layernorm(Exec& ex, const NormW& n, const Act& x, int rows, const Act& y, float dup_scale) {
  if (ex.dry) return;
  LayerNormParams p{};
  p.X = x.p; p.x_dt = x.dt; p.ldx = x.ld; p.Y = y.p; p.y_dt = y.dt; p.ldy = y.ld;
// ... 12 lines not shown
```

Before: 1.437 images/sec.

## Fold nearest-2x upsample into four 2x2 phase convolutions for upsampler convs

```diff
diff --git a/stable-diffusion-xl-burn_amd/csrc/capi_ops.hip b/stable-diffusion-xl-burn_amd/csrc/capi_ops.hip
--- a/stable-diffusion-xl-burn_amd/csrc/capi_ops.hip
+++ b/stable-diffusion-xl-burn_amd/csrc/capi_ops.hip
@@ -325,7 +325,7 @@
   Operands ops;
   add_conv(ops, "conv", Cout, Cin, ksize, weight, bias);
   Packed pk(ops, cdt, s);
-  const Lin l = pk.wb.conv("conv");
+  const Lin l = pk.wb.conv("conv", upsample && ksize == 3 && stride == 1 && pad == 1);
   Tmp tmp;
   void* xi = tmp.get((size_t)B * H * W * Cin * dt_size(sdt));
   float* yo = (float*)tmp.get((size_t)B * Ho * Wo * Cout * sizeof(float));
diff --git a/stable-diffusion-xl-burn_amd/csrc/elementwise.hip b/stable-diffusion-xl-burn_amd/csrc/elementwise.hip
--- a/stable-diffusion-xl-burn_amd/csrc/elementwise.hip
+++ b/stable-diffusion-xl-burn_amd/csrc/elementwise.hip
@@ -798,6 +798,31 @@
   const size_t total = (size_t)Npad * Kpad;
   hipLaunchKernelGGL(pack_conv_kernel, dim3((total + 255) / 256), dim3(256), 0, s, src, dst, dt, Cout, Cin, ks, Kpad, Npad, wscale);
 }
+__global__ void pack_conv_up_phases_kernel(const float* src, void* dst, int dt, int Cout, int Cin, int Kpad, int Npad, float wscale) {
+  const size_t i = (size_t)blockIdx.x * blockDim.x + threadIdx.x;
+  const size_t per = (size_t)Npad * Kpad;
+  if (i >= 4 * per) return;
+  const int ph = (int)(i / per);
+  const size_t r = i - (size_t)ph * per;
+  const int n = (int)(r / Kpad);
+  const int k = (int)(r - (size_t)n * Kpad);
+  float v = 0.f;
+  if (n < Cout && k < 4 * Cin) {
+    const int tap = k / Cin, c = k - tap * Cin;
+    const int py = ph >> 1, px = ph & 1, dy = tap >> 1, dx = tap & 1;
+    const int y0 = py == 0 ? (dy == 0 ? 0 : 1) : (dy == 0 ? 0 : 2), y1 = py == 0 ? (dy == 0 ? 0 : 2) : (dy == 0 ? 1 : 2);
+    const int x0 = px == 0 ? (dx == 0 ? 0 : 1) : (dx == 0 ? 0 : 2), x1 = px == 0 ? (dx == 0 ? 0 : 2) : (dx == 0 ? 1 : 2);
+    const float* w = src + ((size_t)n * Cin + c) * 9;
+    for (int ky = y0; ky <= y1; ++ky)
+      for (int kx = x0; kx <= x1; ++kx) v += w[ky * 3 + kx];
+    v *= wscale;
+  }
+  st_f(dst, i, dt, v);
+}
+void launch_pack_conv_up_phases(const float* src, void* dst, int dt, int Cout, int Cin, int Kpad, int Npad, hipStream_t s, float wscale) {
+  const size_t total = 4 * (size_t)Npad * Kpad;
+  hipLaunchKernelGGL(pack_conv_up_phases_kernel, dim3((unsigned)((total + 255) / 256)), dim3(256), 0, s, src, dst, dt, Cout, Cin, Kpad, Npad, wscale);
+}
 __global__ void pack_bias_kernel(const float* src, float* dst, int N, int Npad, int geglu, int n_offset) {
   const int i = blockIdx.x * blockDim.x + threadIdx.x;
   if (i >= Npad) return;
diff --git a/stable-diffusion-xl-burn_amd/csrc/engine.h b/stable-diffusion-xl-burn_amd/csrc/engine.h
--- a/stable-diffusion-xl-burn_amd/csrc/engine.h
+++ b/stable-diffusion-xl-burn_amd/csrc/engine.h
@@ -111,6 +111,7 @@
   int k_form = 0;
   int dt = -1;
   const float* acc_scale = nullptr;
+  int up_phases = 0;
 };
 struct NormW { const float* gamma = nullptr; const float* beta = nullptr; const float* eps = nullptr; int C = 0; };
 
@@ -133,14 +134,14 @@
   Lin linear(const std::string& name, bool geglu = false, int dt_override = -1);
   Lin fused_linear(const std::vector<std::string>& names, int dt_override = -1);
   Lin linear_hilo(const std::string& name, bool geglu, bool dup = false, bool hl_interleave = false);
-  float hl_scale(Lin& l, const std::vector<std::string>& weight_names);
+  float hl_scale(Lin& l, const std::vector<std::string>& weight_names, int sums_of = 1);
   Lin linear_ln(const std::string& name, bool geglu, const std::string& norm, bool xattn_query = false);
   Lin fused_linear_ln(const std::vector<std::string>& names, const std::string& norm);
   Lin fold_ln(const std::vector<std::string>& names, const std::string& norm, bool geglu, int dt_override = -1, bool shadow = false, Lin* plain = nullptr, bool hilo_dup = false,
               bool hl_interleave = false);
   bool all_f16_exact(const std::vector<std::string>& names);
   float* tmp2 = nullptr; size_t tmp2_numel = 0;
-  Lin conv(const std::string& name);
+  Lin conv(const std::string& name, bool up_phases = false);
   void attach_wfrag(Lin& l, bool fill, bool folded = false);
   NormW norm(const std::string& name);
 };
diff --git a/stable-diffusion-xl-burn_amd/csrc/igemm_common.h b/stable-diffusion-xl-burn_amd/csrc/igemm_common.h
--- a/stable-diffusion-xl-burn_amd/csrc/igemm_common.h
+++ b/stable-diffusion-xl-burn_amd/csrc/igemm_common.h
@@ -143,6 +143,17 @@
   }
 };
 
+template <bool PH>
+__device__ __forceinline__ size_t igemm_out_row(const IgemmParams& p, int m) {
+  if constexpr (!PH) return (size_t)m;
+  else {
+    const int hw = p.Hout * p.Wout;
+    const int b = m / hw, rem = m - b * hw;
+    const int y = rem / p.Wout, x = rem - y * p.Wout;
+    return ((size_t)b * (2 * p.Hout) + (2 * y + p.ph_y)) * (size_t)(2 * p.Wout) + (2 * x + p.ph_x);
+  }
+}
+
 template <int TM, int TN>
 __device__ __forceinline__ void igemm_epilogue(const IgemmParams& p, const f32x16 (&acc)[TM][TN], int mw, int nw, int fr, int fh,
                                                const float (&lnA)[TM], const float (&lnC)[TM]) {
@@ -260,10 +271,11 @@
 }
 
 struct GnCtx { char* scratch; int wave, wm, wn, m0, n0; };
-template <int TM, int TN, bool GEGLU>
+template <int TM, int TN, bool GEGLU, bool PH = false>
 __device__ __forceinline__ void igemm_epilogue_staged_impl(const IgemmParams& p, const f32x16 (&acc)[TM][TN], int mw, int nw,
                                                            int lane, char* lds, bool transposed, const float (&lnA)[TM],
                                                            const float (&lnC)[TM], const void* zeros, const GnCtx* gc = nullptr) {
+  static_assert(!(PH && GEGLU), "phase geometry: plain epilogue only");
   constexpr int WM = TM * 32, WN = TN * 32;
   constexpr int ROWS = WM;
   constexpr int COLS = GEGLU ? WN / 2 : WN;
@@ -435,8 +447,9 @@
 #pragma unroll
         for (int e = 0; e < 8; ++e) rr[e] = p.c_dt == DT_F16 ? (float)(half_t)v[e] : v[e];
       }
+      const size_t mo = igemm_out_row<PH>(p, m);
       if (p.c_dt == DT_F16) {
-        half_t* cp = reinterpret_cast<half_t*>(p.C) + (size_t)m * p.ldc + n0;
+        half_t* cp = reinterpret_cast<half_t*>(p.C) + mo * p.ldc + n0;
         if (full && (reinterpret_cast<uintptr_t>(cp) & 15) == 0) {
           half8 h;
 #pragma unroll
@@ -447,9 +460,9 @@
           for (int e = 0; e < 8; ++e) if (n0 + e < nlim) cp[e] = (half_t)v[e];
         }
       } else if (p.c_dt == DT_HL) {
-        if (full) store_hl8(reinterpret_cast<float*>(p.C) + (size_t)m * p.ldc, n0, v);
+        if (full) store_hl8(reinterpret_cast<float*>(p.C) + mo * p.ldc, n0, v);
       } else {
-        float* cp = reinterpret_cast<float*>(p.C) + (size_t)m * p.ldc + n0;
+        float* cp = reinterpret_cast<float*>(p.C) + mo * p.ldc + n0;
         if (full && (reinterpret_cast<uintptr_t>(cp) & 15) == 0) {
           *reinterpret_cast<f32x4*>(cp) = f32x4{v[0], v[1], v[2], v[3]};
           *reinterpret_cast<f32x4*>(cp + 4) = f32x4{v[4], v[5], v[6], v[7]};
@@ -781,11 +794,15 @@
   }
 }
 
-template <int TM, int TN>
+template <int TM, int TN, bool PH = false>
 __device__ __forceinline__ void igemm_epilogue_staged(const IgemmParams& p, const f32x16 (&acc)[TM][TN], int mw, int nw,
                                                       int lane, char* lds, const float (&lnA)[TM], const float (&lnC)[TM],
                                                       const void* zeros, const GnCtx* gc = nullptr) {
   constexpr int WN = TN * 32;
+  if constexpr (PH) {
+    igemm_epilogue_staged_impl<TM, TN, false, true>(p, acc, mw, nw, lane, lds, false, lnA, lnC, zeros, nullptr);
+    return;
+  }
   if (p.act == 1) { igemm_epilogue_staged_impl<TM, TN, true>(p, acc, mw, nw, lane, lds, false, lnA, lnC, zeros); return; }
   const bool all_normal = nw + WN <= p.n_split || p.n_split >= p.N;
   const bool all_transposed = nw >= p.n_split;
diff --git a/stable-diffusion-xl-burn_amd/csrc/igemm_glds.hip b/stable-diffusion-xl-burn_amd/csrc/igemm_glds.hip
--- a/stable-diffusion-xl-burn_amd/csrc/igemm_glds.hip
+++ b/stable-diffusion-xl-burn_amd/csrc/igemm_glds.hip
@@ -143,9 +143,10 @@
   igemm_epilogue_staged<TM, TN>(p, acc, m0 + wm * WM, n0 + wn * WN, lane, smem + wave * (WM * WN * 4), lnA, lnC, zeros);
 }
 
-template <int BM, int BN, int NS, int WGM = 4, int NW = 8, typename T = half_t, bool XA = false, bool S2 = false, bool TSW = false, bool XH = false>
+template <int BM, int BN, int NS, int WGM = 4, int NW = 8, typename T = half_t, bool XA = false, bool S2 = false, bool TSW = false, bool XH = false, bool PHS = false>
 __global__ __launch_bounds__(64 * NW) void igemm_pipe_kernel(const IgemmParams p, const void* zeros) {
   kernarg_prefetch<(int)sizeof(IgemmParams) + 8>();
+  static_assert(!PHS || (!XA && !S2 && !TSW && !XH), "phase geometry: plain convolution instantiations");
   typedef typename PipeElem<T>::frag frag_t;
   constexpr int CE = 16 / (int)sizeof(T);
   constexpr int WGN = NW / WGM;
@@ -178,6 +179,15 @@
     const int q = nwg >> 3, r = nwg & 7, xcd = bid & 7, idx = bid >> 3;
     bid = (xcd < r ? xcd * (q + 1) : r * (q + 1) + (xcd - r) * q) + idx;
   }
+  const void* Wb = p.W;
+  int ph_y = 0, ph_x = 0;
+  if constexpr (PHS) {
+    const int tiles = tilesM * tilesN;
+    const int phase = __builtin_amdgcn_readfirstlane(bid / tiles);
+    bid -= phase * tiles;
+    Wb = reinterpret_cast<const char*>(p.W) + (size_t)phase * p.ph_wbytes;
+    ph_y = phase >> 1; ph_x = phase & 1;
+  }
   const int SK = p.splitk > 1 ? p.splitk : 1;
   const int slice = SK > 1 ? bid % SK : 0;
   if (SK > 1) bid /= SK;
@@ -203,7 +213,7 @@
 #pragma unroll
   for (int j = 0; j < BJ; ++j) {
     const int row = (j * NW + wave) * 8 + lrow;
-    wptr[j] = reinterpret_cast<const T*>(p.W) + (size_t)(n0 + row) * p.Kpad + (slot ^ ((row >> 1) & 7)) * CE;
+    wptr[j] = reinterpret_cast<const T*>(Wb) + (size_t)(n0 + row) * p.Kpad + (slot ^ ((row >> 1) & 7)) * CE;
   }
   const int nk_all = p.Kpad / KT;
   const int kbeg = SK > 1 ? (int)((long)slice * nk_all / SK) : 0;
@@ -244,6 +254,7 @@
         if (pow2) { b = m >> sh_hw; rem = m & (HWo - 1); oy = rem >> sh_w; }
         else { b = m / HWo; rem = m - b * HWo; oy = rem / p.Wout; }
         rb[j] = b; ry[j] = oy * p.stride - p.pad; rx[j] = (rem - oy * p.Wout) * p.stride - p.pad;
+        if constexpr (PHS) { ry[j] += ph_y; rx[j] += ph_x; }
       } else { rb[j] = -1; ry[j] = -(1 << 28); rx[j] = 0; }
     }
   }
@@ -591,6 +602,13 @@
       __syncthreads();
     }
   }
+  if constexpr (PHS) {
+    static_assert(NW * WM * WN * 4 <= NS * STAGE, "staging regions must fit the dead ring");
+    IgemmParams pe = p;
+    pe.ph_y = ph_y; pe.ph_x = ph_x;
+    igemm_epilogue_staged<TM, TN, true>(pe, acc, m0 + wm * WM, n0 + wn * WN, lane, smem + wave * (WM * WN * 4), lnA, lnC, zeros);
+    return;
+  }
   if constexpr (XA) {
     static_assert(TN == 2 && sizeof(T) == 2, "fused cross-attention: wave tile = one 64-wide head, f16");
     static_assert(NW * WM * WN * 4 <= NS * STAGE, "staging regions must fit the dead ring");
@@ -874,13 +892,14 @@
   hipLaunchKernelGGL((igemm_glds_kernel<BM, BN, NS, MINB>), dim3(c.grid), dim3(c.block), c.lds, s, p, g_zero_pages[dev]);
 }
 
-template <int BM, int BN, int NS, int WGM = 4, int NW = 8, typename T = half_t, bool XA = false, bool S2 = false, bool TSW = false, bool XH = false>
+template <int BM, int BN, int NS, int WGM = 4, int NW = 8, typename T = half_t, bool XA = false, bool S2 = false, bool TSW = false, bool XH = false, bool PHS = false>
 static void launch_pipe(const IgemmParams& p, const IgemmChoice& c, hipStream_t s) {
   if (c.lds != pipe_lds_total(NS * (BM + BN) * 128, 0) || c.block != 64 * NW) throw std::logic_error("igemm: choice and kernel disagree on the LDS layout");
   const int dev = current_device();
-  set_max_dynamic_lds<&igemm_pipe_kernel<BM, BN, NS, WGM, NW, T, XA, S2, TSW, XH>>(c.lds, dev);
+  if (PHS != (p.phases == 4) || (PHS && c.splitk > 1)) throw std::logic_error("igemm: choice and kernel disagree on the phase geometry");
+  set_max_dynamic_lds<&igemm_pipe_kernel<BM, BN, NS, WGM, NW, T, XA, S2, TSW, XH, PHS>>(c.lds, dev);
   if (c.splitk > 1 && (size_t)c.grid * BM * BN * 4 > p.splitk_ws_bytes) throw std::runtime_error("igemm: split-K workspace too small");
-  hipLaunchKernelGGL((igemm_pipe_kernel<BM, BN, NS, WGM, NW, T, XA, S2, TSW, XH>), dim3(c.grid), dim3(c.block), c.lds, s, p, g_zero_pages[dev]);
+  hipLaunchKernelGGL((igemm_pipe_kernel<BM, BN, NS, WGM, NW, T, XA, S2, TSW, XH, PHS>), dim3(c.grid), dim3(c.block), c.lds, s, p, g_zero_pages[dev]);
 }
 
 static void launch_wide(const IgemmParams& p, const IgemmChoice& c, hipStream_t s) {
@@ -927,6 +946,11 @@
 }
 
 void launch_igemm_dma(const IgemmParams& p, const IgemmChoice& c, hipStream_t s) {
+  if (c.ph) {
+    if (c.family == IG_PIPE && c.bm == 256 && c.bn == 128 && c.ns == 3 && c.wgm == 4 && c.nw == 8 && c.elem == DT_HL)
+      return launch_pipe<256, 128, 3, 4, 8, hl16_t, false, false, false, false, true>(p, c, s);
+    throw std::logic_error("igemm: the selection chose a phase-geometry kernel that is not instantiated");
+  }
 #define PIPE(BM, BN, NS, WGM, NW, T, DT, XA, S2, TSW, XH)                                                                                 \
   if (c.family == IG_PIPE && c.bm == BM && c.bn == BN && c.ns == NS && c.wgm == WGM && c.nw == NW && c.elem == DT && c.xa == XA && c.s2 == S2 && c.tsw == TSW && c.xh == XH) \
     return launch_pipe<BM, BN, NS, WGM, NW, T, XA, S2, TSW, XH>(p, c, s)
diff --git a/stable-diffusion-xl-burn_amd/csrc/kernels.h b/stable-diffusion-xl-burn_amd/csrc/kernels.h
--- a/stable-diffusion-xl-burn_amd/csrc/kernels.h
+++ b/stable-diffusion-xl-burn_amd/csrc/kernels.h
@@ -45,6 +45,8 @@
   int epi_staged;
   void* shadow; int shadow_ld; const float* shadow_gamma;
   float shadow_lo_scale;
+  int phases; size_t ph_wbytes;
+  int ph_y, ph_x;
 };
 struct SelectKnobs {
   int igemm_variant = 0;
@@ -68,6 +70,7 @@
   int elem, a_elem;
   int xa, xh, tsw, s2;
   int splitk;
+  int ph;
   int mode, db, measure;
   int grid, block, lds;
 };
@@ -253,6 +256,7 @@
 void launch_beta_dot(const float* w, const float* beta, const float* bias, float* out, int K, int N, hipStream_t s);
 void launch_pack_conv(const float* src, void* dst, int dt, int Cout, int Cin, int ks, int Kpad, int Npad,
                       hipStream_t s, float wscale = 1.0f);
+void launch_pack_conv_up_phases(const float* src, void* dst, int dt, int Cout, int Cin, int Kpad, int Npad, hipStream_t s, float wscale = 1.0f);
 void launch_absmax(const float* src, size_t n, float* out_dev, hipStream_t s, bool accumulate = false);
 void launch_pack_bias(const float* src, float* dst, int N, int Npad, int geglu, int n_offset, hipStream_t s);
 
diff --git a/stable-diffusion-xl-burn_amd/csrc/select.cpp b/stable-diffusion-xl-burn_amd/csrc/select.cpp
--- a/stable-diffusion-xl-burn_amd/csrc/select.cpp
+++ b/stable-diffusion-xl-burn_amd/csrc/select.cpp
@@ -128,7 +128,7 @@
 
 void set_geometry(IgemmChoice& c, const IgemmParams& p) {
   const int tilesM = (p.M + c.bm - 1) / c.bm, tilesN = (p.N + c.bn - 1) / c.bn;
-  c.grid = tilesM * tilesN * (c.splitk > 1 ? c.splitk : 1);
+  c.grid = tilesM * tilesN * (c.splitk > 1 ? c.splitk : 1) * (p.phases ? p.phases : 1);
   switch (c.family) {
     case IG_GLDS: c.block = 256; c.lds = c.ns * (c.bm + c.bn) * 128; break;
     case IG_PIPE: {
@@ -153,6 +153,7 @@
   const Tile& t = tile(number);
   IgemmChoice c{};
   c.family = t.family; c.bm = t.bm; c.bn = t.bn; c.ns = t.ns; c.wgm = t.wgm; c.nw = t.nw; c.s2 = t.s2; c.elem = elem; c.a_elem = elem; c.splitk = 1;
+  c.ph = p.phases != 0;
   set_geometry(c, p);
   return c;
 }
@@ -268,6 +269,7 @@
     if (p.n_split < p.N && ((p.ct_ld & 15) != 0 || (p.rpb & 7) != 0 || (p.M % 8) != 0 || misaligned16(p.Ct))) return false;
   }
   if (p.ebias && (p.ebias_ld & 3) != 0) return false;
+  if (p.phases) { c = from_tile(35, DT_HL, p); return true; }
   const int t96mode = k.hl_tile96;
   const bool splitk = (t96mode & 16) && igemm_splitk_slices(p) > 1;
   const bool plain160 = p.N % 160 == 0 && p.n_split >= p.N && !p.stat_out && p.act == 0;
@@ -312,7 +314,7 @@
 }
 
 int igemm_splitk_slices(const IgemmParams& p) {
-  if (!p.splitk_ws || !p.splitk_cnt) return 1;
+  if (!p.splitk_ws || !p.splitk_cnt || p.phases) return 1;
   if (p.act != 0 || p.n_split < p.N || p.ln_stat) return 1;
   const int nk = p.Kpad / 64;
   if (p.rpb <= 0 || p.rpb > 1024 || p.N > 1536 || nk < 160) return 1;
@@ -330,7 +332,7 @@
   const int kt = hl ? 32 : 64;
   if (hl ? p.c_dt != DT_F32 : (p.a_dt != DT_F16 || p.c_dt != DT_F16)) return false;
   if ((p.Cin % kt) != 0 || (p.lda % (kt / 8)) != 0 || (p.Kpad % kt) != 0) return false;
-  if (p.act != 0 || p.n_split < p.N || p.stat_out || p.ln_stat || p.xa_k) return false;
+  if (p.act != 0 || p.n_split < p.N || p.stat_out || p.ln_stat || p.xa_k || p.phases) return false;
   if (p.M % 256 != 0 || p.rpb <= 0 || p.rpb % 256 != 0 || p.N % 64 != 0) return false;
   if (p.ebias && (p.ebias_ld & 3) != 0) return false;
   if (hl) return (p.ldc & 3) == 0 && !misaligned16(p.C) && (k.hl_tile96 & 16) && igemm_splitk_slices(p) > 1;
@@ -355,6 +357,13 @@
   IgemmChoice c{};
   if (p.M <= 0 || p.N <= 0) return c;
   const int v = k.igemm_variant;
+  if (p.phases) {
+    if (compute_dt != DT_HL) throw std::runtime_error("igemm: phase geometry is the split-operand pipeline's (f16 / fp32 layers are never packed that way)");
+    if (p.phases != 4 || p.ksize != 2 || p.stride != 1 || p.pad != 1 || p.up != 0 || p.Hout != p.Hin || p.Wout != p.Win || p.M != p.B * p.Hin * p.Win || p.K != 4 * p.Cin)
+      throw std::runtime_error("igemm: phase geometry needs the per-phase 2x2-tap GEMM over the source pixels");
+    if (p.gn_part || p.stat_out || p.ln_stat || p.xa_k || p.shadow || p.R || p.act != 0 || p.n_split < p.N)
+      throw std::runtime_error("igemm: phase geometry takes the plain epilogue only (no statistics, residual, activation or split output)");
+  }
   if (compute_dt == DT_F16 && v >= 0 && select_f16(p, v, k, c)) return c;
   if (compute_dt == DT_F16 && v > 0 && select_f16(p, 0, k, c)) return c;
   if (p.shadow && compute_dt != DT_F16) throw std::runtime_error("an f16 shadow output needs an f16 GEMM (weights-in-registers kernel)");
diff --git a/stable-diffusion-xl-burn_amd/csrc/unet.cpp b/stable-diffusion-xl-burn_amd/csrc/unet.cpp
--- a/stable-diffusion-xl-burn_amd/csrc/unet.cpp
+++ b/stable-diffusion-xl-burn_amd/csrc/unet.cpp
@@ -295,7 +295,7 @@
       default:
         b.res = load_res(wb, p + ".res", d.c_in, d.c_out, emb_names, emb_off);
         if (d.kind == BK_REST || d.kind == BK_RESTU) b.st = load_st(wb, p + ".transformer", d.c_out, d.n_head, d.depth, fuse_ln_, plans[sti++]);
-        if (d.kind == BK_RESTU || d.kind == BK_RESU) b.conv = wb.conv(p + ".upsample.conv");
+        if (d.kind == BK_RESTU || d.kind == BK_RESU) b.conv = wb.conv(p + ".upsample.conv", true);
     }
     return b;
   };
diff --git a/stable-diffusion-xl-burn_amd/csrc/vae.cpp b/stable-diffusion-xl-burn_amd/csrc/vae.cpp
--- a/stable-diffusion-xl-burn_amd/csrc/vae.cpp
+++ b/stable-diffusion-xl-burn_amd/csrc/vae.cpp
@@ -42,7 +42,7 @@
       b.r[1] = load_res(wb, p + ".res2", cfg_.dec[i].second, cfg_.dec[i].second);
       b.r[2] = load_res(wb, p + ".res3", cfg_.dec[i].second, cfg_.dec[i].second);
       b.has_up = i + 1 != cfg_.dec.size();
-      if (b.has_up) b.up = wb.conv(p + ".upsampler");
+      if (b.has_up) b.up = wb.conv(p + ".upsampler", true);
       d_blocks_.push_back(b);
     }
     d_norm_out_ = wb.norm("decoder.norm_out");
diff --git a/stable-diffusion-xl-burn_amd/csrc/weights.cpp b/stable-diffusion-xl-burn_amd/csrc/weights.cpp
--- a/stable-diffusion-xl-burn_amd/csrc/weights.cpp
+++ b/stable-diffusion-xl-burn_amd/csrc/weights.cpp
@@ -103,12 +103,19 @@
 }
 WeightBuilder::~WeightBuilder() { if (tmp) (void)hipFree(tmp); if (tmp2) (void)hipFree(tmp2); }
 
+static bool conv_up_phases_ok(int wdt, int ksize, int cin) { return ksize == 3 && wdt == DT_HL && cin % 32 == 0; }
+static bool is_upsampler_conv(const std::string& name) {
+  auto ends = [&](const char* suf) { const std::string t(suf); return name.size() >= t.size() && name.compare(name.size() - t.size(), t.size(), t) == 0; };
+  return ends(".upsample.conv.weight") || ends(".upsampler.weight") || name == "conv.weight";
+}
 size_t WeightBuilder::arena_bound(const std::vector<ParamSpec>& specs, int dt, bool wfrag) {
   size_t total = 1 << 20;
   for (const ParamSpec& p : specs) {
     if (p.kind == PK_LINEAR_W) total += round_up(p.shape[1], 128) * round_up(p.shape[0], 64) * dt_size(dt) + 768;
-    else if (p.kind == PK_CONV_W)
-      total += round_up(p.shape[0], 128) * round_up((size_t)p.shape[1] * p.shape[2] * p.shape[3], 64) * dt_size(dt) + 768;
+    else if (p.kind == PK_CONV_W) {
+      const size_t taps = conv_up_phases_ok(dt, p.shape[2], p.shape[1]) && is_upsampler_conv(p.name) ? 16 : (size_t)p.shape[2] * p.shape[3];
+      total += round_up(p.shape[0], 128) * round_up((size_t)p.shape[1] * taps, 64) * dt_size(dt) + 768;
+    }
     else total += round_up(p.numel(), 128) * sizeof(float) + 256;
     if (p.kind == PK_LINEAR_W || p.kind == PK_CONV_W) total += round_up(p.kind == PK_LINEAR_W ? p.shape[1] : p.shape[0], 128) * 4 + 256;
     if (p.kind == PK_LINEAR_W) total += round_up(p.shape[1], 128) * 4 + 256;
@@ -130,7 +137,7 @@
   last_fetched = name;
   return tmp;
 }
-float WeightBuilder::hl_scale(Lin& l, const std::vector<std::string>& weight_names) {
+float WeightBuilder::hl_scale(Lin& l, const std::vector<std::string>& weight_names, int sums_of) {
   float* sc = (float*)arena.alloc(2 * sizeof(float));
   l.acc_scale = sc;
   if (src.empty()) return 1.f;
@@ -141,10 +148,12 @@
   SDXL_HIP(hipStreamSynchronize(st));
   int e = 0;
   if (h > 0.f && std::isfinite(h)) { (void)std::frexp(h, &e); e = 14 - e; }
+  for (int n = 1; n < sums_of; n *= 2) --e;
   e = e > 24 ? 24 : (e < -24 ? -24 : e);
   const float wscale = std::ldexp(1.0f, e), inv = 1.0f / wscale;
   SDXL_HIP(hipMemcpyAsync(sc, &inv, sizeof(float), hipMemcpyHostToDevice, st));
   SDXL_HIP(hipStreamSynchronize(st));
+  if (sums_of > 1) return wscale;
   bool first = true;
   for (const std::string& n : weight_names) { launch_f16_exact(fetch(n), spec(n).numel(), wscale, sc + 1, st, !first); first = false; }
   return wscale;
@@ -315,10 +324,22 @@
   else launch_colsum_packed(w, dt, l.Kpad, l.Npad, cs, st);
   return l;
 }
-Lin WeightBuilder::conv(const std::string& name) {
+Lin WeightBuilder::conv(const std::string& name, bool up_phases) {
   const ParamSpec& s = spec(name + ".weight");
   Lin l; l.N = s.shape[0]; l.cin = s.shape[1]; l.ksize = s.shape[2];
   l.K = l.cin * l.ksize * l.ksize;
+  if (up_phases && conv_up_phases_ok(dt, l.ksize, l.cin)) {
+    l.up_phases = 4; l.K = 4 * l.cin;
+    l.Kpad = (int)round_up(l.K, 32); l.Npad = (int)round_up(l.N, 128);
+    void* w = arena.alloc(4 * (size_t)l.Npad * l.Kpad * dt_size(dt));
+    float* b = (float*)arena.alloc((size_t)l.Npad * sizeof(float));
+    l.w = w; l.b = b;
+    const float wscale = hl_scale(l, {name + ".weight"}, 4);
+    if (src.empty()) return l;
+    launch_pack_conv_up_phases(fetch(name + ".weight"), w, dt, l.N, l.cin, l.Kpad, l.Npad, st, wscale);
+    launch_pack_bias(fetch(name + ".bias"), b, l.N, l.Npad, 0, 0, st);
+    return l;
+  }
   const int wdt = (dt == DT_HL && l.cin % 32 != 0) ? DT_F32 : dt;
   if (wdt != dt) l.dt = wdt;
   const int kt = wdt == DT_F16 ? 64 : 32;
@@ -386,6 +407,15 @@
   p.M = g.B * g.Hout * g.Wout; p.N = w.N; p.K = w.K; p.Kpad = w.Kpad;
   p.bias = w.b; p.ebias = e.ebias; p.ebias_ld = e.ebias_ld;
   p.rpb = e.rpb ? e.rpb : g.Hout * g.Wout;
+  if (w.up_phases) {
+    SDXL_REQUIRE(g.ksize == 3 && g.stride == 1 && g.pad == 1 && g.up == 1 && g.Hout == 2 * g.Hin && g.Wout == 2 * g.Win,
+                 "run_conv: a phase-packed convolution runs over the nearest-2x image only");
+    SDXL_REQUIRE(!e.R.p && !e.ebias && !e.gn_part && !e.stat_out && !e.ln_stat && !e.xa_k && !e.shadow && e.act == 0 && (e.n_split < 0 || e.n_split >= w.N) && !e.rpb,
+                 "run_conv: the phase form of an upsampler takes the plain epilogue only");
+    p.phases = w.up_phases; p.ph_wbytes = (size_t)w.Npad * w.Kpad * dt_size(ex.cdt);
+    p.Hout = g.Hin; p.Wout = g.Win; p.ksize = 2; p.pad = 1; p.up = 0;
+    p.M = g.B * g.Hin * g.Win; p.rpb = g.Hin * g.Win;
+  }
   p.act = e.act;
   p.R = e.R.p; p.ldr = e.R.ld; p.r_dt = e.R.dt;
   p.C = out.p; p.ldc = out.ld; p.c_dt = out.dt;
@@ -417,11 +447,11 @@
   SDXL_REQUIRE(!e.ln_stat || w.cs, "ln_stat given but the weight is not LayerNorm-folded");
   SDXL_REQUIRE(!w.cs || e.ln_stat, "LayerNorm-folded weight used without row statistics");
   SDXL_REQUIRE(!((w.dt >= 0 ? w.dt : ex.cdt) == DT_F32 && a.dt != DT_F32), "f32 compute needs f32 activations");
-  if (ex.prof) ex.prof->begin(Profiler::IGEMM, 2.0 * p.M * (double)p.N * p.K, ex.s, p.M, p.N, p.K, p.ksize, e.cls);
+  if (ex.prof) ex.prof->begin(Profiler::IGEMM, 2.0 * p.M * (double)p.N * p.K * (p.phases ? p.phases : 1), ex.s, p.M, p.N, p.K, p.ksize, e.cls);
   if (ex.warm && (w.dt >= 0 ? w.dt : ex.cdt) == DT_F16) {
     WarmSeq& ws = *ex.warm;
     const bool host = igemm_wreg_selected(p, knobs) || igemm_wreg_xattn_selected(p, knobs);
-    const size_t wbytes = (size_t)w.Npad * w.Kpad * 2;
+    const size_t wbytes = (size_t)w.Npad * w.Kpad * 2 * (w.up_phases ? w.up_phases : 1);
     const char* lo; const char* hi;
     if (host) {
       const char* f = reinterpret_cast<const char*>(p.Wf), *b = reinterpret_cast<const char*>(w.b);
@@ -458,7 +488,7 @@
     hipStreamCaptureStatus cs = hipStreamCaptureStatusNone;
     if (nan_check && hipStreamIsCapturing(ex.s, &cs) == hipSuccess && cs == hipStreamCaptureStatusNone) {
       const int nout = p.act == 1 ? p.N / 2 : (p.n_split < p.N ? p.n_split : p.N);
-      const unsigned bo = nout > 0 ? count_nonfinite(out.p, out.dt, out.ld, (size_t)p.M, nout, ex.s) : 0;
+      const unsigned bo = nout > 0 ? count_nonfinite(out.p, out.dt, out.ld, (size_t)p.M * (p.phases ? p.phases : 1), nout, ex.s) : 0;
       if (bo) {
         const unsigned bi = p.ksize == 1 && p.stride == 1 && !p.up ? count_nonfinite(a.p, a.dt, a.ld, (size_t)p.M, cin, ex.s) : 0;
         std::fprintf(stderr, "[nan] GEMM tag %d M %d N %d K %d ks %d act %d a_dt %d c_dt %d compute %d: %u non-finite outputs, %u non-finite inputs\n", e.cls, p.M, p.N,
```

After: 1.443 images/sec (median of 6 runs). Within noise of the previous version (+0.4%).
